# Jaureguy760/HaploHyped-VarAwareML

Measured on AMD Instinct MI355X. Metric: variants/sec encode+compress, 3M-variant x 2.5k-sample VCF, higher is better.
Workload: dtype u8

## Files before the change

### haplohyped_varawareml_amd/csrc/api.hip

```cpp
#include "common.h"
#include <chrono>
#include <vector>
#include <stdarg.h>
#include <stdio.h>
#include <string.h>
#include <stdlib.h>

static thread_local char g_err[512] = "";

void hhgt_set_error(const char *fmt, ...)
{
    va_list ap;
    va_start(ap, fmt);
    vsnprintf(g_err, sizeof(g_err), fmt, ap);
    va_end(ap);
}

extern "C" const char *hhgt_last_error(void) { return g_err; }
extern "C" const char *hhgt_version(void) { return "hhgt 0.1 (gfx950)"; }

extern "C" int hhgt_device_count(void)
{
    int n = 0;
    if (hipGetDeviceCount(&n) != hipSuccess) return 0;
    return n;
}

int DevBuf::ensure(size_t bytes)
{
    if (bytes <= cap) return HHGT_OK;
    if (p) {
        hipFree(p);
        p = nullptr;
        cap = 0;
    }
    size_t want = bytes + bytes / 8 + 256;
    static const bool dbg = getenv("HHGT_ALLOC_DEBUG") != nullptr;
    const auto t0 = std::chrono::steady_clock::now();
    hipError_t e = hipMalloc(&p, want);
    if (dbg)
        fprintf(stderr, "[alloc] %.3f ms  hipMalloc %zu took %.3f ms\n", std::chrono::duration<double>(t0.time_since_epoch()).count() * 1e3,
                want, std::chrono::duration<double>(std::chrono::steady_clock::now() - t0).count() * 1e3);
    if (e != hipSuccess) {
        p = nullptr;
        hhgt_set_error("hipMalloc(%zu) failed: %s", want, hipGetErrorString(e));
        return HHGT_ERR_HIP;
    }
    cap = want;
    return HHGT_OK;
}

void DevBuf::release()
{
    if (p) hipFree(p);
    p = nullptr;
    cap = 0;
}

#define TRY(expr)                      \
    do {                               \
        int _rc = (expr);              \
        if (_rc != HHGT_OK) return _rc; \
    } while (0)

int EncodeWs::ensure_index(uint32_t n_regions)
{
    TRY(slots.ensure((size_t)n_regions * INDEX_CAP * 4));
    TRY(counts.ensure((size_t)n_regions * 4));
    TRY(prefix.ensure(((size_t)n_regions + 1) * 4));
    return ensure_scan(n_regions);
}

int EncodeWs::ensure_lines(uint32_t max_lines)
{
    const size_t nl4 = ((size_t)max_lines + 1) * 4;
    TRY(nl.ensure(nl4));
    TRY(ensure_scan(max_lines));
    for (DevBuf &b : line) TRY(b.ensure(nl4));
    return ensure_runs();
}

int EncodeWs::ensure_scan(uint64_t n) { return scan_tmp.ensure(2 * scan_tmp_elems(n) * 4); }

int EncodeWs::ensure_runs()
{
    TRY(run_first.ensure(MAX_CHROM_RUNS * 8));
    TRY(run_names.ensure(MAX_CHROM_RUNS * 32));
    return result.ensure(sizeof(hhgt_encode_result));
}

int hhgt_ctx::CodecWs::ensure(uint64_t n_chunks, uint32_t nblocks, uint32_t nwaves, size_t slot)
{
    const uint64_t n_streams = n_chunks * nblocks * nwaves;
    TRY(lz_scratch.ensure((size_t)n_streams * slot));
    TRY(lz_csize.ensure((size_t)n_streams * 4));
    TRY(fr_bsize.ensure((size_t)n_chunks * nblocks * 4));
    TRY(fr_csize.ensure(((size_t)n_chunks + 1) * 8));
    return fr_flags.ensure((size_t)n_chunks * 4);
}

template <typename Launch>
static int timed(hhgt_ctx *c, hipStream_t st, int stage, Launch launch)
{
    StageTimer t(c, st, stage);
    TRY(launch());
    t.stop();
    return HHGT_OK;
}

extern "C" int hhgt_ctx_create(int device, hhgt_ctx **out)
{
    if (!out) return HHGT_ERR_ARG;
    *out = nullptr;
    int n = hhgt_device_count();
    if (n <= 0 || device < 0 || device >= n) {
        hhgt_set_error("no usable HIP device (count=%d, requested=%d): libhhgt has no CPU path", n, device);
        return HHGT_ERR_NO_DEVICE;
    }
    HIP_TRY(hipSetDevice(device));
    hhgt_ctx *c = new hhgt_ctx();
    c->device = device;
    int rc = HHGT_OK;
    hipError_t e = hipGetDeviceProperties(&c->prop, device);
    if (e != hipSuccess) {
        hhgt_set_error("hipGetDeviceProperties failed: %s", hipGetErrorString(e));
        rc = HHGT_ERR_HIP;
    } else if (strncmp(c->prop.gcnArchName, "gfx950", 6) != 0) {
        hhgt_set_error("device %d is %s; libhhgt carries gfx950 code objects only", device, c->prop.gcnArchName);
        rc = HHGT_ERR_NO_DEVICE;
    }
    if (rc == HHGT_OK && (e = hipHostMalloc(reinterpret_cast<void **>(&c->h_counters), sizeof(DevCounters), hipHostMallocDefault)) != hipSuccess) {
        hhgt_set_error("hipHostMalloc failed: %s", hipGetErrorString(e));
        rc = HHGT_ERR_HIP;
    }
    if (rc == HHGT_OK && (e = hipHostMalloc(reinterpret_cast<void **>(&c->h_result_pinned), sizeof(hhgt_encode_result), hipHostMallocDefault)) != hipSuccess) {
        hhgt_set_error("hipHostMalloc failed: %s", hipGetErrorString(e));
        rc = HHGT_ERR_HIP;
    }
    if (rc == HHGT_OK) rc = c->counters.ensure(sizeof(DevCounters));
    if (rc != HHGT_OK) {
        hhgt_ctx_destroy(c);
        return rc;
    }
    *out = c;
    return HHGT_OK;
}

extern "C" void hhgt_ctx_destroy(hhgt_ctx *c)
{
    if (!c) return;
    hipSetDevice(c->device);
    hipDeviceSynchronize();
    c->enc.each([](DevBuf &b) { b.release(); });
    DevBuf *bufs[] = {&c->counters, &c->cursor, &c->dec_bad, &c->oh_ovl, &c->oh_lut, &c->crc_x2n, &c->ld_bits};
    for (DevBuf *b : bufs) b->release();
    for (auto &w : c->cw) {
        DevBuf *wb[] = {&w.lz_scratch, &w.lz_csize, &w.lz_flags, &w.fr_bsize, &w.fr_csize, &w.fr_flags};
        for (DevBuf *b : wb) b->release();
        if (w.lz_done) hipEventDestroy(w.lz_done);
        if (w.fr_done) hipEventDestroy(w.fr_done);
    }
    if (c->h_counters) hipHostFree(c->h_counters);
    if (c->h_result_pinned) hipHostFree(c->h_result_pinned);
    for (auto &p : c->pending) {
        hipEventDestroy(p.a);
        hipEventDestroy(p.b);
    }
    for (auto e : c->event_pool) hipEventDestroy(e);
    delete c;
}

static hipEvent_t get_event(hhgt_ctx *c)
{
    if (!c->event_pool.empty()) {
        hipEvent_t e = c->event_pool.back();
        c->event_pool.pop_back();
        return e;
    }
    hipEvent_t e;
    hipEventCreate(&e);
    return e;
}

StageTimer::StageTimer(hhgt_ctx *c, hipStream_t s, int stage_) : ctx(c), st(s), stage(stage_)
{
    if (ctx->profiling) {
        a = get_event(ctx);
        b = get_event(ctx);
        hipEventRecord(a, st);
    }
}

void StageTimer::stop()
{
    if (a) {
        hipEventRecord(b, st);
        ctx->pending.push_back({stage, a, b});
        a = b = nullptr;
    }
}

int hhgt_profile_collect(hhgt_ctx *c)
{
    for (auto &p : c->pending) {
        hipEventSynchronize(p.b);
        float ms = 0.f;
        if (hipEventElapsedTime(&ms, p.a, p.b) == hipSuccess) {
            c->stage_ms[p.stage] += ms;
            c->stage_launches[p.stage] += 1;
        }
        c->event_pool.push_back(p.a);
        c->event_pool.push_back(p.b);
    }
    c->pending.clear();
    return HHGT_OK;
}

extern "C" int hhgt_profile_enable(hhgt_ctx *c, int on)
{
    if (!c) return HHGT_ERR_ARG;
    c->profiling = on ? 1 : 0;
    return HHGT_OK;
}

extern "C" int hhgt_profile_reset(hhgt_ctx *c)
{
    if (!c) return HHGT_ERR_ARG;
    hhgt_profile_collect(c);
    for (int i = 0; i < HHGT_N_STAGES; ++i) {
        c->stage_ms[i] = 0;
        c->stage_launches[i] = 0;
    }
    return HHGT_OK;
}

extern "C" int hhgt_profile_read(hhgt_ctx *c, double *ms, uint64_t *launches)
{
    if (!c) return HHGT_ERR_ARG;
    hhgt_profile_collect(c);
    for (int i = 0; i < HHGT_N_STAGES; ++i) {
        if (ms) ms[i] = c->stage_ms[i];
        if (launches) launches[i] = c->stage_launches[i];
    }
    return HHGT_OK;
}

static int make_layout(const hhgt_layout *lay, LayoutDev *L)
{
    if (!lay || lay->n_samples < 0) {
        hhgt_set_error("layout: bad n_samples");
        return HHGT_ERR_ARG;
    }
    L->S = (uint32_t)lay->n_samples;
    L->v_capacity = lay->v_capacity;
    L->ring = 0;
    L->pad_ = 0;
    if (lay->ring < 0 || (lay->ring > 0 && (lay->vc <= 0 || lay->v_capacity != (uint64_t)lay->ring * (uint64_t)lay->vc))) {
        hhgt_set_error("layout: a ring needs vc > 0 and v_capacity == ring * vc");
        return HHGT_ERR_ARG;
    }
    L->ring = (uint32_t)lay->ring;
    if (lay->vc == 0) {
        L->Vc = lay->v_capacity ? lay->v_capacity : TILE_V;
    } else {
        L->Vc = (uint64_t)lay->vc;
    }
    if (L->Vc % TILE_V) {
        hhgt_set_error("layout: variants per chunk (%llu) must be a multiple of %d (dense: v_capacity)",
                       (unsigned long long)L->Vc, TILE_V);
        return HHGT_ERR_ARG;
    }
    if (lay->v_capacity % L->Vc) {
        hhgt_set_error("layout: v_capacity must be a multiple of vc");
        return HHGT_ERR_ARG;
    }
    if (lay->sc == 0) {
        L->Sc = L->S ? L->S : 1;
        L->sc_log2 = 31;
        L->n_sc = 1;
    } else {
        uint32_t sc = (uint32_t)lay->sc;
        if (sc & (sc - 1)) {
            hhgt_set_error("layout: sc must be a power of two");
            return HHGT_ERR_ARG;
        }
        L->Sc = sc;
        uint32_t lg = 0;
        while ((1u << lg) < sc) ++lg;
        L->sc_log2 = lg;
        L->n_sc = (L->S + sc - 1) / sc;
        if (L->n_sc == 0) L->n_sc = 1;
    }
    return HHGT_OK;
}

extern "C" uint64_t hhgt_layout_bytes(const hhgt_layout *lay)
{
    LayoutDev L;
    if (make_layout(lay, &L) != HHGT_OK) return 0;
    return (uint64_t)L.n_sc * L.Sc * L.v_capacity * 2ull;
}

extern "C" uint64_t hhgt_layout_offset(const hhgt_layout *lay, uint32_t s, uint64_t v)
{
    LayoutDev L;
    if (make_layout(lay, &L) != HHGT_OK) return ~0ull;
    return layout_offset(L, s, v);
}

static int parse_region_host(const char *region, RegionFilter *rf)
{
    memset(rf, 0, sizeof(*rf));
    if (!region || !*region) return HHGT_OK;
    const char *colon = strrchr(region, ':');
    size_t clen = strlen(region);
    if (colon && colon[1] >= '0' && colon[1] <= '9') {
        char *p;
        long long b = strtoll(colon + 1, &p, 10), e = 0x7fffffffffffffffLL;
        while (*p == ',') p++;
        if (*p == '-' && p[1]) e = strtoll(p + 1, &p, 10);
        clen = (size_t)(colon - region);
        rf->has_range = 1;
        rf->beg = b;
        rf->end = e;
    }
    if (clen == 0 || clen >= sizeof(rf->contig)) {
        hhgt_set_error("region '%s': contig name empty or longer than 63 bytes", region);
        return HHGT_ERR_ARG;
    }
    memcpy(rf->contig, region, clen);
    rf->contig_len = (int)clen;
    return HHGT_OK;
}

__global__ void k_encode_finish(DevCounters *cnt, uint64_t *cursor, const uint64_t *__restrict__ run_first,
                                const uint8_t *__restrict__ run_names, uint64_t v_capacity, hhgt_encode_result *res)
{
    const uint32_t t = threadIdx.x;
    const uint64_t before = *cursor;
    const uint64_t kept = cnt->n_kept;
    __syncthreads();
    if (t == 0) {
        *cursor = before + kept;
        cnt->cursor_after = before + kept;
        res->stats.n_lines = cnt->n_lines;
        res->stats.n_records = cnt->n_records;
        res->stats.n_kept = kept;
        res->stats.n_drop_region = cnt->n_drop_region;
        res->stats.n_drop_filter = cnt->n_drop_filter;
        res->stats.n_haploid_padded = cnt->n_haploid;
        res->stats.n_malformed = cnt->n_malformed;
        res->stats.n_general_lines = cnt->n_general;
        res->stats.n_chrom_runs = cnt->n_chrom_runs;
        res->cursor_before = before;
        res->cursor_after = before + kept;
        res->n_lines_over = cnt->err_lines;
        res->err_density = cnt->err_density;
        res->v_capacity = v_capacity;
        res->done = 1u;
        res->reserved = cnt->n_other > 0xFFFFFFFFull ? 0xFFFFFFFFu : (uint32_t)cnt->n_other;
    }
    const uint64_t n_runs = cnt->n_chrom_runs;
    if (t < HHGT_RESULT_RUNS) res->run_first[t] = t < n_runs ? run_first[t] : 0ull;
    for (uint32_t q = t; q < HHGT_RESULT_RUNS * 32u; q += blockDim.x)
        res->run_names[q >> 5][q & 31u] = (q >> 5) < n_runs ? (char)run_names[q] : 0;
    __syncthreads();
    if (t < sizeof(DevCounters) / 8u) reinterpret_cast<unsigned long long *>(cnt)[t] = 0ull;
}

__global__ void k_set_u64(uint64_t *p, uint64_t v) { *p = v; }

static int encode_check_args(hhgt_ctx *c, const void *d_text, uint64_t nbytes, const hhgt_layout *lay, LayoutDev *L,
                             const char *region, RegionFilter *rf, void *d_G)
{
    TRY(make_layout(lay, L));
    if (nbytes >= 0xFFFFFFF0ull) {
        hhgt_set_error("encode: text block of %llu bytes; split it below 4 GiB at a line boundary",
                       (unsigned long long)nbytes);
        return HHGT_ERR_ARG;
    }
    if (nbytes && (!d_text || (reinterpret_cast<uintptr_t>(d_text) & 15u))) {
        hhgt_set_error("encode: d_text must be a 16-byte aligned device pointer");
        return HHGT_ERR_ARG;
    }
    if (L->S > 0 && !d_G) {
        hhgt_set_error("encode: d_G is NULL");
        return HHGT_ERR_ARG;
    }
    const int rc = parse_region_host(region, rf);
    rf->keep_multi = c->keep_multi;
    return rc;
}

static uint32_t index_regions(uint64_t nbytes) { return (uint32_t)((nbytes + 1 + INDEX_REGION - 1) / INDEX_REGION); }

static int encode_stage_index(hhgt_ctx *c, const uint8_t *text, uint64_t nbytes, uint32_t n_regions, uint32_t min_line, uint32_t S,
                              DevCounters *cnt, hipStream_t st)
{
    EncodeWs &w = c->enc;
    TRY(w.ensure_index(n_regions));
    TRY(launch_index_newlines(text, nbytes, w.slots.as<uint32_t>(), w.counts.as<uint32_t>(), n_regions, min_line, S, c->index_mode, cnt, st));
    TRY(launch_scan_exclusive_u32_pair(w.counts.as<uint32_t>(), w.prefix.as<uint32_t>(), nullptr, nullptr, n_regions,
                                       w.scan_tmp.as<uint32_t>(), w.scan_tmp.cap / 4, st));
    return HHGT_OK;
}

static int encode_stage_rest(hhgt_ctx *c, const uint8_t *text, uint64_t nbytes, uint32_t n_regions, uint32_t max_lines,
                             const RegionFilter &rf, const LayoutDev &L, const uint64_t *d_cursor, void *d_G, void *d_P, uint32_t *d_start, uint32_t *d_stop,
                             uint8_t *d_ref, uint8_t *d_alt, DevCounters *cnt, hipStream_t st)
{
    EncodeWs &w = c->enc;
    TRY(w.ensure_lines(max_lines));
    const uint32_t *nl = w.nl.as<uint32_t>(), *d_nlines = w.prefix.as<uint32_t>() + n_regions;
    uint32_t *scan_tmp = w.scan_tmp.as<uint32_t>();
    const LineCols l = w.line_cols();
    const KeptCols k = w.kept_cols();
    TRY(timed(c, st, HHGT_STAGE_INDEX, [&] {
        return launch_compact_newlines(w.slots.as<uint32_t>(), w.counts.as<uint32_t>(), w.prefix.as<uint32_t>(), n_regions,
                                       w.nl.as<uint32_t>(), max_lines, st);
    }));
    if (max_lines == 0) return HHGT_OK;
    TRY(timed(c, st, HHGT_STAGE_FIXED, [&] {
        TRY(launch_parse_fixed(text, nbytes, nl, d_nlines, max_lines, rf, L.S, l, c->index_mode, cnt, st));
        TRY(launch_scan_exclusive_u32_pair(l.keep, l.kidx, l.cnew, l.crun, max_lines, scan_tmp, w.scan_tmp.cap / 4, st));
        return launch_compact_kept(text, nbytes, nl, d_nlines, max_lines, l, k, MAX_CHROM_RUNS, d_cursor, L.v_capacity, L.ring,
                                   d_start, d_stop, d_ref, d_alt, cnt, d_P != nullptr, st);
    }));
    if (L.S == 0) return HHGT_OK;
    TRY(timed(c, st, HHGT_STAGE_ENCODE, [&] {
        return d_P ? launch_encode_planes(text, nbytes, k.soff, k.meta, max_lines, d_cursor, L, static_cast<uint8_t *>(d_P),
                                          static_cast<int8_t *>(d_G), k.redo_list, k.redo_flag, cnt, st)
                   : launch_encode_tiles(text, nbytes, k.soff, k.meta, max_lines, d_cursor, L, static_cast<int8_t *>(d_G),
                                         k.redo_list, k.redo_flag, cnt, st);
    }));
    return timed(c, st, HHGT_STAGE_GENERAL, [&] {
        return launch_encode_general(text, nbytes, k.soff, k.lend, k.meta, k.redo_list, d_cursor, L, static_cast<int8_t *>(d_G),
                                     static_cast<uint8_t *>(d_P), cnt, c->prop.multiProcessorCount, st);
    });
}

static int encode_finish(hhgt_ctx *c, uint64_t *d_cursor, const LayoutDev &L, DevCounters *cnt, hipStream_t st)
{
    TRY(c->enc.ensure_runs());
    const KeptCols k = c->enc.kept_cols();
    hipLaunchKernelGGL(k_encode_finish, dim3(1), dim3(256), 0, st, cnt, d_cursor, k.run_first, k.run_names,
                       L.ring ? 0ull : L.v_capacity, c->enc.result.as<hhgt_encode_result>());
    HIP_TRY(hipGetLastError());
    return HHGT_OK;
}

extern "C" int hhgt_encode_result_status(const hhgt_encode_result *r)
{
    if (!r) return HHGT_ERR_ARG;
    if (!r->done) {
        hhgt_set_error("encode: the result record is not complete yet (synchronise the stream first)");
        return HHGT_ERR_ARG;
    }
    if (r->err_density) {
        hhgt_set_error("encode: more than %u newlines inside one %u-byte region (not VCF text)", INDEX_CAP, INDEX_REGION);
        return HHGT_ERR_LINE_DENSITY;
    }
    if (r->n_lines_over) {
        hhgt_set_error("encode: %llu lines beyond max_lines were not encoded", (unsigned long long)r->n_lines_over);
        return HHGT_ERR_CAPACITY;
    }
    if (r->stats.n_malformed) {
        hhgt_set_error("Error parsing VCF file: %llu malformed record(s) (too few columns, bad POS, FORMAT without GT)",
                       (unsigned long long)r->stats.n_malformed);
        return HHGT_ERR_MALFORMED;
    }
    if (r->v_capacity && r->cursor_after > r->v_capacity) {
        hhgt_set_error("encode: %llu kept records at v_base %llu exceed v_capacity %llu",
                       (unsigned long long)r->stats.n_kept, (unsigned long long)r->cursor_before,
                       (unsigned long long)r->v_capacity);
        return HHGT_ERR_CAPACITY;
    }
    if (r->stats.n_chrom_runs > MAX_CHROM_RUNS) {
        hhgt_set_error("encode: %llu CHROM runs in one text block, more than the limit of %u (a run starts at every change of CHROM "
                       "and behind every empty or header line)",
                       (unsigned long long)r->stats.n_chrom_runs, MAX_CHROM_RUNS);
        return HHGT_ERR_CAPACITY;
    }
    return HHGT_OK;
}

static void empty_result(hhgt_encode_result *r)
{
    memset(r, 0, sizeof(*r));
    r->done = 1u;
}

static int planes_check_layout(const LayoutDev &L)
{
    if (L.Vc % 4096ull) {
        hhgt_set_error("planes: variants per chunk (%llu; dense: v_capacity) must be a multiple of 4096", (unsigned long long)L.Vc);
        return HHGT_ERR_ARG;
    }
    return HHGT_OK;
}

extern "C" uint64_t hhgt_planes_bytes(const hhgt_layout *lay)
{
    LayoutDev L;
    if (make_layout(lay, &L) != HHGT_OK || planes_check_layout(L) != HHGT_OK) return 0;
    return (uint64_t)L.n_sc * L.Sc * L.v_capacity / 2ull;
}

static int planes_columns(const hhgt_layout *lay, uint32_t col0, uint32_t n_cols, LayoutDev *L, PlanesGeom *pg)
{
    TRY(make_layout(lay, L));
    TRY(planes_check_layout(*L));
    if ((uint64_t)col0 + n_cols > L->v_capacity / L->Vc) {
        hhgt_set_error("planes: columns [%u, %u) outside the layout's %llu", col0, col0 + n_cols, (unsigned long long)(L->v_capacity / L->Vc));
        return HHGT_ERR_ARG;
    }
    *pg = planes_geom(*L, col0);
    return HHGT_OK;
}

static int pad_tail_begin(hhgt_ctx *c, const void *d_buf, const hhgt_layout *lay, bool planes, LayoutDev *L)
{
    if (!c || !d_buf) return HHGT_ERR_ARG;
    HIP_TRY(hipSetDevice(c->device));
    TRY(make_layout(lay, L));
    return planes ? planes_check_layout(*L) : HHGT_OK;
}

static int pad_tail_range(const LayoutDev &L, uint64_t v_end, uint64_t vcol_end)
{
    if (v_end > L.v_capacity || vcol_end > L.v_capacity / L.Vc) {
        hhgt_set_error("pad_tail: range outside the layout");
        return HHGT_ERR_ARG;
    }
    return HHGT_OK;
}

static int encode_async_impl(hhgt_ctx *c, const void *d_text, uint64_t nbytes, const char *region, const hhgt_layout *lay,
                             uint64_t *d_cursor, uint32_t max_lines, void *d_G, void *d_P, bool planes, uint32_t *d_start,
                             uint32_t *d_stop, uint8_t *d_ref, uint8_t *d_alt, hhgt_encode_result *h_result, void *stream)
{
    if (!c || !d_cursor) return HHGT_ERR_ARG;
    hipStream_t st = reinterpret_cast<hipStream_t>(stream);
    HIP_TRY(hipSetDevice(c->device));
    LayoutDev L;
    RegionFilter rf;
    TRY(encode_check_args(c, d_text, nbytes, lay, &L, region, &rf, planes ? d_P : d_G));
    if (planes) TRY(planes_check_layout(L));
    const uint8_t *text = static_cast<const uint8_t *>(d_text);
    DevCounters *cnt = c->counters.as<DevCounters>();
    if (!c->counters_clean) HIP_TRY(hipMemsetAsync(cnt, 0, sizeof(DevCounters), st));
    c->counters_clean = false;
    const uint32_t n_regions = index_regions(nbytes);
    if (nbytes) {
        TRY(timed(c, st, HHGT_STAGE_INDEX, [&] { return encode_stage_index(c, text, nbytes, n_regions, L.S ? 2u * L.S + 17u : 0u, L.S, cnt, st); }));
        TRY(encode_stage_rest(c, text, nbytes, n_regions, max_lines, rf, L, d_cursor, d_G, planes ? d_P : nullptr, d_start, d_stop, d_ref,
                              d_alt, cnt, st));
    }
    TRY(encode_finish(c, d_cursor, L, cnt, st));
    c->counters_clean = true;
    if (h_result) {
        h_result->done = 0u;
        HIP_TRY(hipMemcpyAsync(h_result, c->enc.result.p, sizeof(hhgt_encode_result), hipMemcpyDeviceToHost, st));
    }
    return HHGT_OK;
}

extern "C" int hhgt_encode_text_async(hhgt_ctx *c, const void *d_text, uint64_t nbytes, const char *region,
                                      const hhgt_layout *lay, uint64_t *d_cursor, uint32_t max_lines, void *d_G,
                                      uint32_t *d_start, uint32_t *d_stop, uint8_t *d_ref, uint8_t *d_alt,
                                      hhgt_encode_result *h_result, void *stream)
{
    return encode_async_impl(c, d_text, nbytes, region, lay, d_cursor, max_lines, d_G, nullptr, false, d_start, d_stop, d_ref, d_alt,
                             h_result, stream);
}

extern "C" int hhgt_encode_text_planes_async(hhgt_ctx *c, const void *d_text, uint64_t nbytes, const char *region,
                                             const hhgt_layout *lay, uint64_t *d_cursor, uint32_t max_lines, void *d_P, void *d_G,
                                             uint32_t *d_start, uint32_t *d_stop, uint8_t *d_ref, uint8_t *d_alt,
                                             hhgt_encode_result *h_result, void *stream)
{
    return encode_async_impl(c, d_text, nbytes, region, lay, d_cursor, max_lines, d_G, d_P, true, d_start, d_stop, d_ref, d_alt,
                             h_result, stream);
}

extern "C" int hhgt_pad_tail_planes(hhgt_ctx *c, const hhgt_layout *lay, uint64_t v_end, uint64_t vcol_begin, uint64_t vcol_end,
                                    void *d_P, void *stream)
{
    LayoutDev L;
    TRY(pad_tail_begin(c, d_P, lay, true, &L));
    TRY(pad_tail_range(L, v_end, vcol_end));
    return launch_pad_tail_planes(L, v_end, vcol_begin, vcol_end, static_cast<uint8_t *>(d_P), reinterpret_cast<hipStream_t>(stream));
}

extern "C" int hhgt_pad_tail_planes_cursor(hhgt_ctx *c, const hhgt_layout *lay, const uint64_t *d_cursor, void *d_P, void *stream)
{
    LayoutDev L;
    if (!d_cursor) return HHGT_ERR_ARG;
    TRY(pad_tail_begin(c, d_P, lay, true, &L));
    return launch_pad_tail_planes_cursor(L, d_cursor, static_cast<uint8_t *>(d_P), reinterpret_cast<hipStream_t>(stream));
}

extern "C" int hhgt_planes_expand(hhgt_ctx *c, const hhgt_layout *lay, const void *d_P, const void *d_G, uint32_t col0, uint32_t n_cols,
                                  void *d_out, void *stream)
{
    if (!c || !d_P || !d_out) return HHGT_ERR_ARG;
    HIP_TRY(hipSetDevice(c->device));
    LayoutDev L;
    PlanesGeom pg;
    TRY(planes_columns(lay, col0, n_cols, &L, &pg));
    if (n_cols == 0) return HHGT_OK;
    return launch_planes_expand(L, static_cast<const uint8_t *>(d_P), static_cast<const uint8_t *>(d_G), col0, n_cols,
                                static_cast<uint8_t *>(d_out), reinterpret_cast<hipStream_t>(stream));
}

static int encode_text_once(hhgt_ctx *c, const void *d_text, uint64_t nbytes, const char *region, const hhgt_layout *lay, uint64_t v_base,
                            void *d_G, uint32_t *d_start, uint32_t *d_stop, uint8_t *d_ref, uint8_t *d_alt, hhgt_encode_stats *stats,
                            void *stream);

extern "C" int hhgt_encode_text(hhgt_ctx *c, const void *d_text, uint64_t nbytes, const char *region,
                                const hhgt_layout *lay, uint64_t v_base, void *d_G, uint32_t *d_start,
                                uint32_t *d_stop, uint8_t *d_ref, uint8_t *d_alt, hhgt_encode_stats *stats,
                                void *stream)
{
    int rc = encode_text_once(c, d_text, nbytes, region, lay, v_base, d_G, d_start, d_stop, d_ref, d_alt, stats, stream);
    if (rc == HHGT_ERR_MALFORMED && c && lay && lay->n_samples >= 760) {
        const int mode = c->index_mode < 0 ? index_mode_default() : c->index_mode;
        if (mode > 0) {
            const int saved = c->index_mode;
            c->index_mode = 0;
            rc = encode_text_once(c, d_text, nbytes, region, lay, v_base, d_G, d_start, d_stop, d_ref, d_alt, stats, stream);
            c->index_mode = saved;
        }
    }
    return rc;
}

static int encode_text_once(hhgt_ctx *c, const void *d_text, uint64_t nbytes, const char *region, const hhgt_layout *lay, uint64_t v_base,
                            void *d_G, uint32_t *d_start, uint32_t *d_stop, uint8_t *d_ref, uint8_t *d_alt, hhgt_encode_stats *stats,
                            void *stream)
{
    if (!c) return HHGT_ERR_ARG;
    hipStream_t st = reinterpret_cast<hipStream_t>(stream);
    HIP_TRY(hipSetDevice(c->device));
    if (stats) memset(stats, 0, sizeof(*stats));
    LayoutDev L;
    RegionFilter rf;
    TRY(encode_check_args(c, d_text, nbytes, lay, &L, region, &rf, d_G));
    c->run_first_kept.clear();
    c->run_names_host.clear();
    if (nbytes == 0) return HHGT_OK;

    const uint8_t *text = static_cast<const uint8_t *>(d_text);
    DevCounters *cnt = c->counters.as<DevCounters>();
    TRY(c->cursor.ensure(8));
    HIP_TRY(hipMemsetAsync(cnt, 0, sizeof(DevCounters), st));
    c->counters_clean = false;
    hipLaunchKernelGGL(k_set_u64, dim3(1), dim3(1), 0, st, c->cursor.as<uint64_t>(), v_base);
    const uint32_t n_regions = index_regions(nbytes);
    uint32_t n_lines = 0;
    {
        StageTimer t(c, st, HHGT_STAGE_INDEX);
        TRY(encode_stage_index(c, text, nbytes, n_regions, L.S ? 2u * L.S + 17u : 0u, L.S, cnt, st));
        c->h_counters->n_lines = 0;
        c->h_counters->err_density = 0;
        HIP_TRY(hipMemcpyAsync(&c->h_counters->n_lines, c->enc.prefix.as<uint32_t>() + n_regions, 4,
                               hipMemcpyDeviceToHost, st));
        HIP_TRY(hipMemcpyAsync(&c->h_counters->err_density, &cnt->err_density, 8, hipMemcpyDeviceToHost, st));
        HIP_TRY(hipStreamSynchronize(st));
        t.stop();
        n_lines = (uint32_t)(c->h_counters->n_lines & 0xFFFFFFFFull);
        if (c->h_counters->err_density) {
            hhgt_set_error("encode: more than %u newlines inside one %u-byte region (not VCF text)", INDEX_CAP,
                           INDEX_REGION);
            return HHGT_ERR_LINE_DENSITY;
        }
    }
    if (stats) stats->n_lines = n_lines;
    if (n_lines == 0) return HHGT_OK;
    TRY(encode_stage_rest(c, text, nbytes, n_regions, n_lines, rf, L, c->cursor.as<uint64_t>(), d_G, nullptr, d_start, d_stop, d_ref,
                          d_alt, cnt, st));
    TRY(encode_finish(c, c->cursor.as<uint64_t>(), L, cnt, st));
    c->counters_clean = true;
    hhgt_encode_result *hr = &c->h_result;
    hr->done = 0u;
    HIP_TRY(hipMemcpyAsync(c->h_result_pinned, c->enc.result.p, sizeof(hhgt_encode_result), hipMemcpyDeviceToHost, st));
    HIP_TRY(hipStreamSynchronize(st));
    *hr = *c->h_result_pinned;
    if (stats) *stats = hr->stats;
    TRY(hhgt_encode_result_status(hr));
    const uint32_t n_runs = (uint32_t)hr->stats.n_chrom_runs;
    if (n_runs) {
        std::vector<uint64_t> first(n_runs);
        std::vector<char> names((size_t)n_runs * 32);
        if (n_runs <= HHGT_RESULT_RUNS) {
            memcpy(first.data(), hr->run_first, n_runs * 8);
            memcpy(names.data(), hr->run_names, (size_t)n_runs * 32);
        } else {
            HIP_TRY(hipMemcpy(first.data(), c->enc.run_first.p, (size_t)n_runs * 8, hipMemcpyDeviceToHost));
            HIP_TRY(hipMemcpy(names.data(), c->enc.run_names.p, (size_t)n_runs * 32, hipMemcpyDeviceToHost));
        }
        for (uint32_t r = 0; r < n_runs; ++r) {
            c->run_first_kept.push_back(first[r]);
            c->run_names_host.emplace_back(names.data() + (size_t)r * 32, strnlen(names.data() + (size_t)r * 32, 31));
        }
    }
    return HHGT_OK;
}

extern "C" int hhgt_encode_chrom_runs(hhgt_ctx *c, uint32_t max_runs, uint64_t *first_kept, char *names,
                                      uint32_t *n_runs)
{
    if (!c || !n_runs) return HHGT_ERR_ARG;
    uint32_t n = (uint32_t)c->run_first_kept.size();
    *n_runs = n;
    if (n > max_runs) n = max_runs;
    for (uint32_t r = 0; r < n; ++r) {
        if (first_kept) first_kept[r] = c->run_first_kept[r];
        if (names) {
            memset(names + (size_t)r * 32, 0, 32);
            size_t l = c->run_names_host[r].size() < 31 ? c->run_names_host[r].size() : 31;
            memcpy(names + (size_t)r * 32, c->run_names_host[r].data(), l);
        }
    }
    return HHGT_OK;
}

extern "C" int hhgt_pad_tail(hhgt_ctx *c, const hhgt_layout *lay, uint64_t v_end, uint64_t vcol_begin,
                             uint64_t vcol_end, void *d_G, void *stream)
{
    LayoutDev L;
    TRY(pad_tail_begin(c, d_G, lay, false, &L));
    TRY(pad_tail_range(L, v_end, vcol_end));
    return launch_pad_tail(L, v_end, vcol_begin, vcol_end, static_cast<int8_t *>(d_G),
                           reinterpret_cast<hipStream_t>(stream));
}

extern "C" int hhgt_pad_tail_cursor(hhgt_ctx *c, const hhgt_layout *lay, const uint64_t *d_cursor, void *d_G, void *stream)
{
    LayoutDev L;
    if (!d_cursor) return HHGT_ERR_ARG;
    TRY(pad_tail_begin(c, d_G, lay, false, &L));
    return launch_pad_tail_cursor(L, d_cursor, static_cast<int8_t *>(d_G), reinterpret_cast<hipStream_t>(stream));
}

static int check_codec_args(uint64_t chunk_nbytes, int typesize, int blocksize, int format)
{
    if (typesize < 1 || typesize > 255 || blocksize < 16 || blocksize > 65536 || blocksize % typesize ||
        chunk_nbytes == 0 || chunk_nbytes >= 0x7fffffffull || (format != HHGT_BLOSC1 && format != HHGT_BLOSC2)) {
        hhgt_set_error("compress: bad arguments (chunk_nbytes=%llu typesize=%d blocksize=%d format=%d)",
                       (unsigned long long)chunk_nbytes, typesize, blocksize, format);
        return HHGT_ERR_ARG;
    }
    return HHGT_OK;
}

static int effective_blocksize(uint64_t chunk_nbytes, int typesize, int blocksize)
{
    if ((uint64_t)blocksize > chunk_nbytes) {
        blocksize = (int)chunk_nbytes;
        if (typesize > 1 && blocksize >= typesize) blocksize -= blocksize % typesize;
    }
    return blocksize > 0 ? blocksize : 1;
}

static int check_decode_block(int typesize, int blocksize)
{
    if (blocksize > 65536) {
        hhgt_set_error("decode: block of %d bytes x typesize %d does not fit LDS (blocks of at most 65536 bytes)",
                       blocksize, typesize);
        return HHGT_ERR_ARG;
    }
    return HHGT_OK;
}

static void codec_geometry(uint64_t chunk_nbytes, int typesize, int blocksize, uint32_t *nblocks, uint32_t *nwaves,
                           size_t *slot_bytes)
{
    const bool split = typesize >= 2 && typesize <= 16 && blocksize / typesize >= 128;
    *nblocks = (uint32_t)((chunk_nbytes + blocksize - 1) / blocksize);
    *nwaves = split ? (uint32_t)typesize : 1u;
    size_t max_stream = split ? (size_t)blocksize / typesize : (size_t)blocksize;
    if (split && chunk_nbytes % blocksize && chunk_nbytes % blocksize > max_stream) max_stream = chunk_nbytes % blocksize;
    *slot_bytes = lz4_slot_bytes((int)max_stream);
}

extern "C" uint64_t hhgt_compress_bound(uint64_t n_chunks, uint64_t chunk_nbytes, int typesize, int blocksize)
{
    if (check_codec_args(chunk_nbytes, typesize, blocksize, HHGT_BLOSC2) != HHGT_OK) return 0;
    return n_chunks * (chunk_nbytes + 32);
}

static int compress_impl(hhgt_ctx *c, const void *d_src, const void *d_planes, PlanesGeom pg, uint64_t n_chunks, uint64_t chunk_nbytes,
                         int typesize, int blocksize, int format, void *d_dst, uint64_t dst_cap,
                         uint64_t *d_chunk_off, uint64_t *total_bytes, void *stream)
{
    if (!c || (!d_src && !d_planes) || !d_dst || !d_chunk_off) return HHGT_ERR_ARG;
    hipStream_t st = reinterpret_cast<hipStream_t>(stream);
    HIP_TRY(hipSetDevice(c->device));
    TRY(check_codec_args(chunk_nbytes, typesize, blocksize, format));
    if (total_bytes) *total_bytes = 0;
    if (n_chunks == 0) return HHGT_OK;
    if (!total_bytes && dst_cap < n_chunks * (chunk_nbytes + 32)) {
        hhgt_set_error("compress: the asynchronous form (total_bytes == NULL) needs dst_cap >= hhgt_compress_bound() = %llu, got %llu",
                       (unsigned long long)(n_chunks * (chunk_nbytes + 32)), (unsigned long long)dst_cap);
        return HHGT_ERR_CAPACITY;
    }
    blocksize = effective_blocksize(chunk_nbytes, typesize, blocksize);
    uint32_t nblocks, nwaves;
    size_t slot;
    codec_geometry(chunk_nbytes, typesize, blocksize, &nblocks, &nwaves, &slot);
    hipStream_t fst = c->frame_stream ? c->frame_stream : st;
    hhgt_ctx::CodecWs &w = c->cw[c->frame_stream ? (c->cmp_seq++ & 1u) : 0u];
    TRY(w.ensure(n_chunks, nblocks, nwaves, slot));
    if (w.fr_pending) {
        HIP_TRY(hipStreamWaitEvent(st, w.fr_done, 0));
        w.fr_pending = false;
    }
    TRY(timed(c, st, HHGT_STAGE_LZ4, [&] {
        if (!w.lz_flags.p) {
            TRY(w.lz_flags.ensure(4));
            HIP_TRY(hipMemsetAsync(w.lz_flags.p, 0, 4, st));
        }
        if (++w.lz_tag == 0) w.lz_tag = 1;
        return launch_lz4_blocks(static_cast<const uint8_t *>(d_src), static_cast<const uint8_t *>(d_planes), pg, n_chunks, chunk_nbytes,
                                 typesize, blocksize, w.lz_scratch.as<uint8_t>(), slot, w.lz_csize.as<uint32_t>(), c->clevel,
                                 w.lz_flags.as<uint32_t>(), w.lz_tag, st);
    }));
    if (fst != st) {
        if (!w.lz_done) HIP_TRY(hipEventCreateWithFlags(&w.lz_done, hipEventDisableTiming));
        if (!w.fr_done) HIP_TRY(hipEventCreateWithFlags(&w.fr_done, hipEventDisableTiming));
        HIP_TRY(hipEventRecord(w.lz_done, st));
        HIP_TRY(hipStreamWaitEvent(fst, w.lz_done, 0));
    }
    TRY(timed(c, fst, HHGT_STAGE_FRAME, [&] {
        return launch_frame(w.lz_scratch.as<uint8_t>(), slot, w.lz_csize.as<uint32_t>(), static_cast<const uint8_t *>(d_src),
                            static_cast<const uint8_t *>(d_planes), pg, n_chunks, chunk_nbytes, typesize, blocksize, format,
                            w.fr_bsize.as<uint32_t>(), w.fr_csize.as<uint64_t>(), static_cast<uint8_t *>(d_dst), dst_cap, d_chunk_off,
                            w.fr_flags.as<uint32_t>(), fst);
    }));
    if (fst != st) {
        HIP_TRY(hipEventRecord(w.fr_done, fst));
        w.fr_pending = true;
        if (total_bytes) HIP_TRY(hipStreamWaitEvent(st, w.fr_done, 0));
    }
    if (total_bytes) {
        uint64_t tot = 0;
        HIP_TRY(hipMemcpyAsync(&tot, d_chunk_off + n_chunks, 8, hipMemcpyDeviceToHost, st));
        HIP_TRY(hipStreamSynchronize(st));
        *total_bytes = tot;
        if (tot > dst_cap) {
            hhgt_set_error("compress: need %llu bytes, dst_cap is %llu", (unsigned long long)tot,
                           (unsigned long long)dst_cap);
            return HHGT_ERR_CAPACITY;
        }
    }
    return HHGT_OK;
}

extern "C" int hhgt_compress_chunks(hhgt_ctx *c, const void *d_src, uint64_t n_chunks, uint64_t chunk_nbytes,
                                    int typesize, int blocksize, int format, void *d_dst, uint64_t dst_cap,
                                    uint64_t *d_chunk_off, uint64_t *total_bytes, void *stream)
{
    if (!d_src) return HHGT_ERR_ARG;
    return compress_impl(c, d_src, nullptr, PlanesGeom{0, 0, 0, 0}, n_chunks, chunk_nbytes, typesize, blocksize, format, d_dst, dst_cap,
                         d_chunk_off, total_bytes, stream);
}

extern "C" int hhgt_compress_planes(hhgt_ctx *c, const hhgt_layout *lay, const void *d_P, const void *d_G, uint32_t col0, uint32_t n_cols,
                                    int format, void *d_dst, uint64_t dst_cap, uint64_t *d_chunk_off, uint64_t *total_bytes,
                                    void *stream)
{
    if (!c || !d_P) return HHGT_ERR_ARG;
    LayoutDev L;
    PlanesGeom pg;
    TRY(planes_columns(lay, col0, n_cols, &L, &pg));
    const uint64_t chunk_nbytes = (uint64_t)L.Sc * L.Vc * 2ull, col_bytes = chunk_nbytes * L.n_sc;
    const uint8_t *g = d_G ? static_cast<const uint8_t *>(d_G) + (uint64_t)col0 * col_bytes : nullptr;
    return compress_impl(c, g, d_P, pg, (uint64_t)n_cols * L.n_sc, chunk_nbytes, 2, 8192, format, d_dst, dst_cap, d_chunk_off, total_bytes,
                         stream);
}

extern "C" int hhgt_reserve(hhgt_ctx *c, uint64_t text_bytes, uint32_t max_lines, uint64_t n_chunks, uint64_t chunk_nbytes, int typesize,
                            int blocksize)
{
    if (!c) return HHGT_ERR_ARG;
    HIP_TRY(hipSetDevice(c->device));
    if (text_bytes) {
        const uint32_t n_regions = index_regions(text_bytes);
        TRY(c->enc.ensure_scan(n_regions > max_lines ? n_regions : max_lines));
        TRY(c->enc.ensure_index(n_regions));
        TRY(c->enc.ensure_lines(max_lines));
    }
    if (n_chunks) {
        TRY(check_codec_args(chunk_nbytes, typesize, blocksize, HHGT_BLOSC2));
        blocksize = effective_blocksize(chunk_nbytes, typesize, blocksize);
        uint32_t nblocks, nwaves;
        size_t slot;
        codec_geometry(chunk_nbytes, typesize, blocksize, &nblocks, &nwaves, &slot);
        TRY(c->cw[0].ensure(n_chunks, nblocks, nwaves, slot));
    }
    return HHGT_OK;
}

extern "C" int hhgt_set_clevel(hhgt_ctx *c, int clevel)
{
    if (!c || clevel < 1 || clevel > 9) {
        hhgt_set_error("clevel must be 1..9");
        return HHGT_ERR_ARG;
    }
    c->clevel = clevel;
    return HHGT_OK;
}

extern "C" int hhgt_stream_create(hhgt_ctx *c, int kind, void **out)
{
    if (!c || !out || (kind != HHGT_STREAM_ENCODE && kind != HHGT_STREAM_COMPRESS && kind != HHGT_STREAM_FRAME)) {
        hhgt_set_error("hhgt_stream_create: bad arguments");
        return HHGT_ERR_ARG;
    }
    HIP_TRY(hipSetDevice(c->device));
    hipStream_t st = nullptr;
    if (kind == HHGT_STREAM_FRAME) {
        HIP_TRY(hipStreamCreateWithFlags(&st, hipStreamNonBlocking));
    } else if (kind == HHGT_STREAM_ENCODE) {
        int lo = 0, hi = 0;
        HIP_TRY(hipDeviceGetStreamPriorityRange(&lo, &hi));
        HIP_TRY(hipStreamCreateWithPriority(&st, hipStreamNonBlocking, hi));
    } else {
        const uint32_t n_cu = (uint32_t)c->prop.multiProcessorCount;
        uint32_t use = n_cu >= 128u ? (n_cu * 3u / 4u) / 32u * 32u : n_cu;
        if (const char *e = getenv("HHGT_COMPRESS_CUS")) {
            const int v = atoi(e);
            use = v <= 0 || (uint32_t)v >= n_cu ? n_cu : (uint32_t)v;
        }
        if (use >= n_cu) {
            HIP_TRY(hipStreamCreateWithFlags(&st, hipStreamNonBlocking));
        } else {
            std::vector<uint32_t> mask((n_cu + 31u) / 32u, 0u);
            for (uint32_t i = n_cu - use; i < n_cu; ++i) mask[i >> 5] |= 1u << (i & 31u);
            if (hipExtStreamCreateWithCUMask(&st, (uint32_t)mask.size(), mask.data()) != hipSuccess) {
                (void)hipGetLastError();
                st = nullptr;
                HIP_TRY(hipStreamCreateWithFlags(&st, hipStreamNonBlocking));
            }
        }
    }
    *out = st;
    return HHGT_OK;
}

extern "C" int hhgt_set_frame_stream(hhgt_ctx *c, void *stream)
{
    if (!c) return HHGT_ERR_ARG;
    HIP_TRY(hipSetDevice(c->device));
    if (c->frame_stream) HIP_TRY(hipStreamSynchronize(c->frame_stream));
    for (auto &w : c->cw) w.fr_pending = false;
    c->frame_stream = reinterpret_cast<hipStream_t>(stream);
    return HHGT_OK;
}

extern "C" int hhgt_stream_destroy(hhgt_ctx *c, void *stream)
{
    if (!c) return HHGT_ERR_ARG;
    if (stream) {
        HIP_TRY(hipSetDevice(c->device));
        if (reinterpret_cast<hipStream_t>(stream) == c->frame_stream) TRY(hhgt_set_frame_stream(c, nullptr));
        HIP_TRY(hipStreamDestroy(reinterpret_cast<hipStream_t>(stream)));
    }
    return HHGT_OK;
}

extern "C" int hhgt_set_index_mode(hhgt_ctx *c, int mode)
{
    if (!c || mode < -1 || mode > 2) {
        hhgt_set_error("index mode must be -1 (default), 0 (scan), 1 (hop) or 2 (walk)");
        return HHGT_ERR_ARG;
    }
    c->index_mode = mode;
    return HHGT_OK;
}

extern "C" int hhgt_set_keep_multiallelic(hhgt_ctx *c, int on)
{
    if (!c) return HHGT_ERR_ARG;
    c->keep_multi = on ? 1 : 0;
    return HHGT_OK;
}

__global__ void k_count_nonzero_u32(const uint32_t *__restrict__ v, uint64_t n, unsigned long long *out)
{
    uint64_t i = (uint64_t)blockIdx.x * blockDim.x + threadIdx.x;
    const unsigned long long m = __ballot(i < n && v[i] != 0u);
    if ((threadIdx.x & 63u) == 0u && m) atomicAdd(out, (unsigned long long)__builtin_popcountll(m));
}

extern "C" int hhgt_inflate_members(hhgt_ctx *c, const void *d_src, uint64_t src_bytes, const uint64_t *d_comp_off,
                                    const uint32_t *d_comp_len, const uint64_t *d_out_off, const uint32_t *d_isize,
                                    uint64_t n_members, void *d_dst, uint64_t dst_bytes, const uint32_t *d_crc32,
                                    uint32_t *d_status, uint64_t *n_bad, void *stream)
{
    if (!c || !d_src || !d_comp_off || !d_comp_len || !d_out_off || !d_isize || !d_status || (!d_dst && dst_bytes))
        return HHGT_ERR_ARG;
    hipStream_t st = reinterpret_cast<hipStream_t>(stream);
    HIP_TRY(hipSetDevice(c->device));
    if (n_bad) *n_bad = 0;
    if (n_members == 0) return HHGT_OK;
    if (d_crc32 && !c->crc_x2n_ready) {
        uint32_t t[32];
        crc32_x2n_table(t);
        TRY(c->crc_x2n.ensure(sizeof(t)));
        HIP_TRY(hipMemcpy(c->crc_x2n.p, t, sizeof(t), hipMemcpyHostToDevice));
        c->crc_x2n_ready = true;
    }
    TRY(timed(c, st, HHGT_STAGE_INFLATE, [&] {
        return launch_inflate(static_cast<const uint8_t *>(d_src), src_bytes, d_comp_off, d_comp_len, d_out_off, d_isize, n_members,
                              static_cast<uint8_t *>(d_dst), dst_bytes, d_status, d_crc32, c->crc_x2n.as<uint32_t>(), st);
    }));
    if (n_bad) {
        TRY(c->dec_bad.ensure(8));
        HIP_TRY(hipMemsetAsync(c->dec_bad.p, 0, 8, st));
        hipLaunchKernelGGL(k_count_nonzero_u32, dim3((uint32_t)((n_members + 255) / 256)), dim3(256), 0, st, d_status,
                           n_members, c->dec_bad.as<unsigned long long>());
        HIP_TRY(hipGetLastError());
        uint64_t nb = 0;
        HIP_TRY(hipMemcpyAsync(&nb, c->dec_bad.p, 8, hipMemcpyDeviceToHost, st));
        HIP_TRY(hipStreamSynchronize(st));
        *n_bad = nb;
    }
    return HHGT_OK;
}

template <typename Launch>
static int with_bad_counter(hhgt_ctx *c, hipStream_t st, uint64_t *n_bad, Launch launch)
{
    TRY(c->dec_bad.ensure(8));
    HIP_TRY(hipMemsetAsync(c->dec_bad.p, 0, 8, st));
    TRY(timed(c, st, HHGT_STAGE_DECODE, [&] { return launch(c->dec_bad.as<unsigned long long>()); }));
    if (n_bad) {
        uint64_t nb = 0;
        HIP_TRY(hipMemcpyAsync(&nb, c->dec_bad.p, 8, hipMemcpyDeviceToHost, st));
        HIP_TRY(hipStreamSynchronize(st));
        *n_bad = nb;
    }
    return HHGT_OK;
}

extern "C" int hhgt_decompress_chunks(hhgt_ctx *c, const void *d_src, const uint64_t *d_chunk_off, uint64_t n_chunks,
                                      uint64_t chunk_nbytes, int typesize, int blocksize, void *d_dst,
                                      uint64_t *n_bad, void *stream)
{
    if (!c || !d_src || !d_dst || !d_chunk_off) return HHGT_ERR_ARG;
    hipStream_t st = reinterpret_cast<hipStream_t>(stream);
    HIP_TRY(hipSetDevice(c->device));
    TRY(check_decode_block(typesize, blocksize));
    TRY(check_codec_args(chunk_nbytes, typesize, blocksize, HHGT_BLOSC2));
    if (n_bad) *n_bad = 0;
    if (n_chunks == 0) return HHGT_OK;
    blocksize = effective_blocksize(chunk_nbytes, typesize, blocksize);
    return with_bad_counter(c, st, n_bad, [&](unsigned long long *d_bad) {
        return launch_decode(static_cast<const uint8_t *>(d_src), d_chunk_off, n_chunks, chunk_nbytes, typesize, blocksize,
                             static_cast<uint8_t *>(d_dst), d_bad, st);
    });
}

extern "C" int hhgt_decompress_blocks(hhgt_ctx *c, const hhgt_block_sel *d_sel, uint32_t n_sel, uint64_t chunk_nbytes,
                                      int typesize, int blocksize, void *d_dst, uint64_t *n_bad, void *stream)
{
    if (!c || (n_sel && (!d_sel || !d_dst))) {
        hhgt_set_error("decompress_blocks: null %s", !c ? "context" : !d_sel ? "selection array" : "destination");
        return HHGT_ERR_ARG;
    }
    hipStream_t st = reinterpret_cast<hipStream_t>(stream);
    HIP_TRY(hipSetDevice(c->device));
    TRY(check_decode_block(typesize, blocksize));
    TRY(check_codec_args(chunk_nbytes, typesize, blocksize, HHGT_BLOSC2));
    if (n_bad) *n_bad = 0;
    if (n_sel == 0) return HHGT_OK;
    blocksize = effective_blocksize(chunk_nbytes, typesize, blocksize);
    return with_bad_counter(c, st, n_bad, [&](unsigned long long *d_bad) {
        return launch_decode_sel(d_sel, n_sel, chunk_nbytes, typesize, blocksize, static_cast<uint8_t *>(d_dst), d_bad, st);
    });
}

static int check_row_kernel_args(const char *who, uint32_t sc, uint32_t vc, int typesize, int blocksize)
{
    if (typesize != 2) {
        hhgt_set_error("%s: typesize %d (only 2: one diploid int8 call)", who, typesize);
        return HHGT_ERR_ARG;
    }
    if (sc < 1 || sc > 64 || vc < 1) {
        hhgt_set_error("%s: chunk of %u samples x %u variants (1 to 64 samples)", who, sc, vc);
        return HHGT_ERR_ARG;
    }
    TRY(check_codec_args((uint64_t)sc * vc * 2u, typesize, blocksize, HHGT_BLOSC2));
    if (blocksize > 8192 || ((uint64_t)vc * 2u) % (uint64_t)blocksize) {
        hhgt_set_error("%s: blocksize %d does not cut a row of %u variants into whole blocks of at most 8192 bytes", who,
                       blocksize, vc);
        return HHGT_ERR_ARG;
    }
    return HHGT_OK;
}

template <typename Launch>
static int run_row_kernel(const char *who, const char *out, hhgt_ctx *c, const void *d_sel, uint32_t n_sel, const void *d_out,
                          uint32_t sc, uint32_t vc, int typesize, int blocksize, uint64_t *n_bad, void *stream, Launch launch)
{
    if (!c || (n_sel && (!d_sel || !d_out))) {
        hhgt_set_error("%s: null %s", who, !c ? "context" : !d_sel ? "selection array" : out);
        return HHGT_ERR_ARG;
    }
    TRY(check_row_kernel_args(who, sc, vc, typesize, blocksize));
    hipStream_t st = reinterpret_cast<hipStream_t>(stream);
    HIP_TRY(hipSetDevice(c->device));
    if (n_bad) *n_bad = 0;
    if (n_sel == 0) return HHGT_OK;
    return with_bad_counter(c, st, n_bad, [&](unsigned long long *d_bad) { return launch(d_bad, st); });
}

extern "C" int hhgt_count_alleles(hhgt_ctx *c, const hhgt_count_sel *d_sel, uint32_t n_sel, uint32_t sc, uint32_t vc,
                                  int typesize, int blocksize, uint32_t *d_counts, uint64_t n_out, uint64_t *n_bad,
                                  void *stream)
{
    return run_row_kernel("count_alleles", "counts", c, d_sel, n_sel, d_counts, sc, vc, typesize, blocksize, n_bad, stream,
                          [&](unsigned long long *d_bad, hipStream_t st) {
                              return launch_count_alleles(d_sel, n_sel, sc, vc, blocksize, d_counts, n_out, d_bad, st);
                          });
}

extern "C" int hhgt_count_samples(hhgt_ctx *c, const hhgt_sample_sel *d_sel, uint32_t n_sel, uint32_t sc, uint32_t vc,
                                  int typesize, int blocksize, const uint32_t *d_vmask, uint64_t vmask_words,
                                  uint32_t *d_counts, uint64_t n_out, uint64_t *n_bad, void *stream)
{
    return run_row_kernel("count_samples", "counts", c, d_sel, n_sel, d_counts, sc, vc, typesize, blocksize, n_bad, stream,
                          [&](unsigned long long *d_bad, hipStream_t st) {
                              return launch_count_samples(d_sel, n_sel, sc, vc, blocksize, d_vmask, vmask_words, d_counts,
                                                          n_out, d_bad, st);
                          });
}

extern "C" int hhgt_genotype_planes(hhgt_ctx *c, const hhgt_plane_sel *d_sel, uint32_t n_sel, uint32_t sc, uint32_t vc,
                                    int typesize, int blocksize, const uint32_t *d_vmask, uint64_t vmask_words,
                                    uint32_t *d_planes, uint64_t n_rows, uint64_t row_words, uint64_t *n_bad,
                                    void *stream)
{
    return run_row_kernel("genotype_planes", "planes", c, d_sel, n_sel, d_planes, sc, vc, typesize, blocksize, n_bad, stream,
                          [&](unsigned long long *d_bad, hipStream_t st) {
                              return launch_genotype_planes(d_sel, n_sel, sc, vc, blocksize, d_vmask, vmask_words, d_planes,
                                                            n_rows, row_words, d_bad, st);
                          });
}

template <typename Launch>
static int run_plane_kernel(const char *who, int stage, hhgt_ctx *c, const char *null_arg, const char *misaligned, uint64_t n_rows,
                            uint64_t row_words, uint64_t w_lo, uint64_t w_hi, uint64_t row_limit, void *stream, Launch launch)
{
    const bool work = n_rows && w_lo < w_hi;
    if (!c || (work && null_arg)) {
        hhgt_set_error("%s: null %s", who, !c ? "context" : null_arg);
        return HHGT_ERR_ARG;
    }
    if (w_lo > w_hi || w_hi > row_words || n_rows > row_limit) {
        hhgt_set_error("%s: words [%llu, %llu) of rows of %llu words, %llu rows", who, (unsigned long long)w_lo,
                       (unsigned long long)w_hi, (unsigned long long)row_words, (unsigned long long)n_rows);
        return HHGT_ERR_ARG;
    }
    if (misaligned) {
        hhgt_set_error("%s: %s", who, misaligned);
        return HHGT_ERR_ARG;
    }
    hipStream_t st = reinterpret_cast<hipStream_t>(stream);
    HIP_TRY(hipSetDevice(c->device));
    if (!work) return HHGT_OK;
    return timed(c, st, stage, [&] { return launch(st); });
}

static bool off_alignment(const void *p, uintptr_t align) { return reinterpret_cast<uintptr_t>(p) & (align - 1u); }

extern "C" int hhgt_pair_counts(hhgt_ctx *c, const uint32_t *d_planes, uint64_t n_rows, uint64_t row_words, uint64_t w_lo,
                                uint64_t w_hi, uint32_t *d_table, void *stream)
{
    return run_plane_kernel("pair_counts", HHGT_STAGE_PAIRS, c, !d_planes ? "planes" : !d_table ? "table" : nullptr,
                            off_alignment(d_table, 16) ? "the table must be 16-byte aligned" : nullptr, n_rows, row_words, w_lo, w_hi,
                            64ull * 65535ull, stream, [&](hipStream_t st) {
                                return launch_pair_counts(d_planes, (uint32_t)n_rows, row_words, w_lo, w_hi, d_table, st);
                            });
}

extern "C" int hhgt_grm(hhgt_ctx *c, const uint32_t *d_planes, uint64_t n_rows, uint64_t row_words, uint64_t w_lo, uint64_t w_hi,
                        const float *d_z, double *d_table, void *stream)
{
    return run_plane_kernel("grm", HHGT_STAGE_GRM, c, !d_planes ? "planes" : !d_z ? "weights" : !d_table ? "table" : nullptr,
                            off_alignment(d_table, 8) || off_alignment(d_z, 16)
                                ? "the table must be 8-byte aligned, the weights 16-byte aligned" : nullptr,
                            n_rows, row_words, w_lo, w_hi, 64ull * 65535ull, stream, [&](hipStream_t st) {
                                return launch_grm(d_planes, (uint32_t)n_rows, row_words, w_lo, w_hi, d_z, d_table, st);
                            });
}

extern "C" int hhgt_variant_planes(hhgt_ctx *c, const uint32_t *d_planes, uint64_t n_rows, uint64_t row_words, uint64_t w_lo,
                                   uint64_t w_hi, uint32_t *d_vplanes, void *stream)
{
    return run_plane_kernel("variant_planes", HHGT_STAGE_LD_TRANSPOSE, c, !d_planes ? "planes" : !d_vplanes ? "variant planes" : nullptr,
                            nullptr, n_rows, row_words, w_lo, w_hi, 256ull * 65535ull, stream, [&](hipStream_t st) {
                                return launch_variant_planes(d_planes, (uint32_t)n_rows, row_words, w_lo, w_hi, d_vplanes, st);
                            });
}

static int check_ld_args(const char *who, hhgt_ctx *c, uint32_t window, const double *r2, const char *null_arg, const uint32_t *d_table)
{
    if (window < 1u || window > 1024u || (r2 && !(*r2 >= 0.0 && *r2 <= 1.0))) {
        if (r2)
            hhgt_set_error("%s: window %u, r2 %g (1 to 1024, 0 to 1)", who, window, *r2);
        else
            hhgt_set_error("%s: window %u (1 to 1024)", who, window);
        return HHGT_ERR_ARG;
    }
    if (!c || null_arg) {
        hhgt_set_error("%s: null %s", who, !c ? "context" : null_arg);
        return HHGT_ERR_ARG;
    }
    if (off_alignment(d_table, 32)) {
        hhgt_set_error("%s: the table must be 32-byte aligned", who);
        return HHGT_ERR_ARG;
    }
    return HHGT_OK;
}

extern "C" int hhgt_ld_counts(hhgt_ctx *c, const uint32_t *d_vplanes, uint64_t n_var, uint64_t sw, uint32_t window,
                              uint32_t *d_table, void *stream)
{
    const bool work = n_var && sw;
    TRY(check_ld_args("ld_counts", c, window, nullptr, !work ? nullptr : !d_vplanes ? "variant planes" : !d_table ? "table" : nullptr, d_table));
    hipStream_t st = reinterpret_cast<hipStream_t>(stream);
    HIP_TRY(hipSetDevice(c->device));
    if (!work) return HHGT_OK;
    return timed(c, st, HHGT_STAGE_LD, [&] { return launch_ld_counts(d_vplanes, n_var, sw, window, d_table, st); });
}

extern "C" int hhgt_ld_prune(hhgt_ctx *c, const uint32_t *d_table, uint64_t n_var, uint32_t window, double r2,
                             uint8_t *d_keep, void *stream)
{
    TRY(check_ld_args("ld_prune", c, window, &r2, !n_var ? nullptr : !d_table ? "table" : !d_keep ? "keep flags" : nullptr, d_table));
    hipStream_t st = reinterpret_cast<hipStream_t>(stream);
    HIP_TRY(hipSetDevice(c->device));
    if (!n_var) return HHGT_OK;
    TRY(c->ld_bits.ensure((size_t)n_var * ld_walk_words(window) * sizeof(uint64_t)));
    uint64_t *bits = c->ld_bits.as<uint64_t>();
    TRY(timed(c, st, HHGT_STAGE_LD_PRUNE, [&] { return launch_ld_exceeds(d_table, n_var, window, r2, bits, st); }));
    return timed(c, st, HHGT_STAGE_LD_WALK, [&] { return launch_ld_walk(bits, n_var, window, d_keep, st); });
}

extern "C" int hhgt_assoc_sums(hhgt_ctx *c, const uint32_t *d_vplanes, uint64_t n_var, uint64_t sw, const double *d_w,
                               uint32_t n_cols, double *d_sums, void *stream)
{
    if (n_cols < 1u || n_cols > 64u) {
        hhgt_set_error("assoc_sums: %u columns (1 to 64)", n_cols);
        return HHGT_ERR_ARG;
    }
    const bool reads = n_var && sw;
    const char *null_arg = !n_var ? nullptr : !d_sums ? "sums" : !reads ? nullptr : !d_vplanes ? "variant planes" : !d_w ? "weights" : nullptr;
    if (!c || null_arg) {
        hhgt_set_error("assoc_sums: null %s", !c ? "context" : null_arg);
        return HHGT_ERR_ARG;
    }
    if (off_alignment(d_w, 8) || off_alignment(d_sums, 8)) {
        hhgt_set_error("assoc_sums: the weights and the sums must be 8-byte aligned");
        return HHGT_ERR_ARG;
    }
    hipStream_t st = reinterpret_cast<hipStream_t>(stream);
    HIP_TRY(hipSetDevice(c->device));
    if (!n_var) return HHGT_OK;
    return timed(c, st, HHGT_STAGE_ASSOC, [&] { return launch_assoc_sums(d_vplanes, n_var, sw, d_w, n_cols, d_sums, st); });
}
```

### haplohyped_varawareml_amd/csrc/common.h

```cpp
#pragma once
#include <hip/hip_runtime.h>
#include <stdint.h>
#include <stddef.h>
#include <string>
#include <vector>
#include "../../include/hhgt.h"

#define HHGT_WAVE 64
#ifdef HHGT_ENC_PRIO
#define HHGT_WAVE_PRIO() __builtin_amdgcn_s_setprio(HHGT_ENC_PRIO)
#else
#define HHGT_WAVE_PRIO()
#endif

#ifdef __HIPCC__
__device__ __forceinline__ uint32_t wave_scan_sum_dpp(uint32_t x, uint32_t lane)
{
    x += (uint32_t)__builtin_amdgcn_update_dpp(0, (int)x, 0x111, 0xf, 0xf, false);
    x += (uint32_t)__builtin_amdgcn_update_dpp(0, (int)x, 0x112, 0xf, 0xf, false);
    x += (uint32_t)__builtin_amdgcn_update_dpp(0, (int)x, 0x114, 0xf, 0xf, false);
    x += (uint32_t)__builtin_amdgcn_update_dpp(0, (int)x, 0x118, 0xf, 0xf, false);
    const uint32_t t0 = (uint32_t)__builtin_amdgcn_readlane((int)x, 15);
    const uint32_t t1 = (uint32_t)__builtin_amdgcn_readlane((int)x, 31) + t0;
    const uint32_t t2 = (uint32_t)__builtin_amdgcn_readlane((int)x, 47) + t1;
    const uint32_t row = lane >> 4;
    return x + (row == 0u ? 0u : (row == 1u ? t0 : (row == 2u ? t1 : t2)));
}
#endif

void hhgt_set_error(const char *fmt, ...);
#define HIP_TRY(expr)                                                                      \
    do {                                                                                   \
        hipError_t _e = (expr);                                                            \
        if (_e != hipSuccess) {                                                            \
            hhgt_set_error("%s failed: %s (%s:%d)", #expr, hipGetErrorString(_e), __FILE__, \
                           __LINE__);                                                      \
            return HHGT_ERR_HIP;                                                           \
        }                                                                                  \
    } while (0)

enum : uint32_t {
    LF_RECORD = 1u,
    LF_KEEP = 2u,
    LF_FAST = 4u,
    LF_MALFORMED = 8u,
    LF_DROP_REGION = 16u,
    LF_DROP_FILTER = 32u,
    LF_CHROM_NEW = 64u,
};

struct DevCounters {
    unsigned long long n_lines;
    unsigned long long n_records;
    unsigned long long n_kept;
    unsigned long long n_drop_region;
    unsigned long long n_drop_filter;
    unsigned long long n_haploid;
    unsigned long long n_malformed;
    unsigned long long n_general;
    unsigned long long n_chrom_runs;
    unsigned long long err_density;
    unsigned long long err_lines;
    unsigned long long cursor_after;
    unsigned long long n_other;
    unsigned long long pad[3];
};

#define MAX_CHROM_RUNS 4096u

struct RegionFilter {
    char contig[64];
    int contig_len;
    int has_range;
    long long beg, end;
    int keep_multi;
};

#define INDEX_REGION 16384u
#define INDEX_CAP 1024u

#define TILE_V 128
#define TILE_S 256

struct LayoutDev {
    uint32_t S;
    uint32_t sc_log2;
    uint32_t n_sc;
    uint32_t Sc;
    uint64_t Vc;
    uint64_t v_capacity;
    uint32_t ring;
    uint32_t pad_;
};

#define PL_TILE 256u
struct PlanesGeom {
    uint32_t S_pad;
    uint32_t bpr;
    uint32_t tpc;
    uint32_t col0;
};
static inline __host__ __device__ uint64_t planes_piece(const PlanesGeom &g, uint64_t col, uint32_t tile, uint32_t kp, uint32_t row)
{
    return ((((col * g.tpc + tile) * 4ull + kp) * g.S_pad) + row) * 32ull;
}
static inline __host__ __device__ PlanesGeom planes_geom(const LayoutDev &L, uint32_t col0)
{
    PlanesGeom g;
    g.S_pad = L.n_sc * L.Sc;
    g.bpr = (uint32_t)(L.Vc >> 12);
    g.tpc = (uint32_t)(L.Vc / PL_TILE);
    g.col0 = col0;
    return g;
}
static inline __host__ __device__ void planes_block(const PlanesGeom &g, uint64_t id, uint64_t *col, uint32_t *row, uint32_t *bi)
{
    const uint64_t per_col = (uint64_t)g.S_pad * g.bpr;
    const uint64_t c = id / per_col;
    const uint32_t rem = (uint32_t)(id - c * per_col);
    *col = g.col0 + c;
    *row = rem / g.bpr;
    *bi = rem - (rem / g.bpr) * g.bpr;
}

struct DevBuf {
    void *p = nullptr;
    size_t cap = 0;
    int ensure(size_t bytes);
    void release();
    template <typename T> T *as() const { return reinterpret_cast<T *>(p); }
};

struct LineCols {
    uint32_t *soff, *lend, *pos, *refalt, *flags, *keep, *kidx, *cnew, *crun;
};
struct KeptCols {
    uint32_t *soff, *lend, *meta, *redo_list, *redo_flag;
    uint64_t *run_first;
    uint8_t *run_names;
};

struct EncodeWs {
    DevBuf slots, counts, prefix, nl, scan_tmp;
    enum { L_SOFF, L_LEND, L_POS, L_REFALT, L_FLAGS, L_KEEP, L_KIDX, L_CNEW, L_CRUN, K_SOFF, K_LEND, K_META, REDO_LIST, REDO_FLAG, N_LINE };
    DevBuf line[N_LINE];
    DevBuf run_first, run_names;
    DevBuf result;
    int ensure_index(uint32_t n_regions);
    int ensure_lines(uint32_t max_lines);
    int ensure_scan(uint64_t n);
    int ensure_runs();
    template <typename F> void each(F f)
    {
        for (DevBuf *b : {&slots, &counts, &prefix, &nl, &scan_tmp, &run_first, &run_names, &result}) f(*b);
        for (DevBuf &b : line) f(b);
    }
    uint32_t *col(int i) const { return line[i].as<uint32_t>(); }
    LineCols line_cols() const
    {
        LineCols l;
        l.soff = col(L_SOFF), l.lend = col(L_LEND), l.pos = col(L_POS), l.refalt = col(L_REFALT), l.flags = col(L_FLAGS);
        l.keep = col(L_KEEP), l.kidx = col(L_KIDX), l.cnew = col(L_CNEW), l.crun = col(L_CRUN);
        return l;
    }
    KeptCols kept_cols() const
    {
        KeptCols k;
        k.soff = col(K_SOFF), k.lend = col(K_LEND), k.meta = col(K_META), k.redo_list = col(REDO_LIST), k.redo_flag = col(REDO_FLAG);
        k.run_first = run_first.as<uint64_t>(), k.run_names = run_names.as<uint8_t>();
        return k;
    }
};

struct hhgt_ctx {
    int device = 0;
    hipDeviceProp_t prop;
    EncodeWs enc;
    DevBuf counters;
    DevBuf cursor;
    struct CodecWs {
        DevBuf lz_scratch, lz_csize, lz_flags, fr_bsize, fr_csize, fr_flags;
        uint32_t lz_tag = 0;
        hipEvent_t lz_done = nullptr, fr_done = nullptr;
        bool fr_pending = false;
        int ensure(uint64_t n_chunks, uint32_t nblocks, uint32_t nwaves, size_t slot);
    } cw[2];
    uint64_t cmp_seq = 0;
    hipStream_t frame_stream = nullptr;
    DevBuf dec_bad, oh_ovl, oh_lut, crc_x2n;
    DevBuf ld_bits;
    bool crc_x2n_ready = false;
    DevCounters *h_counters = nullptr;
    hhgt_encode_result *h_result_pinned = nullptr;
    hhgt_encode_result h_result;
    std::vector<uint64_t> run_first_kept;
    std::vector<std::string> run_names_host;
    int clevel = 5;
    int keep_multi = 0;
    int index_mode = -1;
    bool counters_clean = false;
    int profiling = 0;
    double stage_ms[HHGT_N_STAGES] = {0};
    uint64_t stage_launches[HHGT_N_STAGES] = {0};
    struct Pending { int stage; hipEvent_t a, b; };
    std::vector<Pending> pending;
    std::vector<hipEvent_t> event_pool;
};

struct StageTimer {
    hhgt_ctx *ctx;
    hipStream_t st;
    int stage;
    hipEvent_t a = nullptr, b = nullptr;
    StageTimer(hhgt_ctx *c, hipStream_t s, int stage_);
    void stop();
};
int hhgt_profile_collect(hhgt_ctx *ctx);

int launch_scan_exclusive_u32(const uint32_t *d_in, uint32_t *d_out, uint64_t n, uint32_t *d_tmp,
                              size_t tmp_elems, hipStream_t st);
int launch_scan_exclusive_u32_pair(const uint32_t *in_a, uint32_t *out_a, const uint32_t *in_b, uint32_t *out_b, uint64_t n,
                                   uint32_t *d_tmp, size_t tmp_elems, hipStream_t st);
size_t scan_tmp_elems(uint64_t n);

int launch_index_newlines(const uint8_t *d_text, uint64_t n, uint32_t *d_slots, uint32_t *d_counts,
                          uint32_t n_regions, uint32_t min_line, uint32_t S, int mode, DevCounters *d_cnt, hipStream_t st);
int index_mode_default();
int launch_compact_newlines(const uint32_t *d_slots, const uint32_t *d_counts, const uint32_t *d_prefix,
                            uint32_t n_regions, uint32_t *d_nl, uint32_t max_lines, hipStream_t st);
int launch_parse_fixed(const uint8_t *d_text, uint64_t n, const uint32_t *d_nl, const uint32_t *d_nlines,
                       uint32_t max_lines, const RegionFilter &region, uint32_t S, const LineCols &l, int mode,
                       DevCounters *d_cnt, hipStream_t st);
int launch_compact_kept(const uint8_t *d_text, uint64_t n, const uint32_t *d_nl, const uint32_t *d_nlines, uint32_t max_lines,
                        const LineCols &l, const KeptCols &k, uint32_t max_runs, const uint64_t *d_cursor, uint64_t v_capacity,
                        uint32_t ring, uint32_t *d_start, uint32_t *d_stop, uint8_t *d_ref, uint8_t *d_alt, DevCounters *d_cnt,
                        bool strided, hipStream_t st);

int launch_encode_tiles(const uint8_t *d_text, uint64_t n, const uint32_t *k_soff, const uint32_t *k_meta,
                        uint32_t n_lines_bound, const uint64_t *d_cursor, LayoutDev lay, int8_t *d_G,
                        uint32_t *redo_list, uint32_t *redo_flag, DevCounters *d_cnt, hipStream_t st);
int launch_encode_general(const uint8_t *d_text, uint64_t n, const uint32_t *k_soff, const uint32_t *k_lend,
                          const uint32_t *k_meta, const uint32_t *redo_list, const uint64_t *d_cursor, LayoutDev lay,
                          int8_t *d_G, uint8_t *d_P, DevCounters *d_cnt, int n_cu, hipStream_t st);
int launch_encode_planes(const uint8_t *d_text, uint64_t n, const uint32_t *k_soff, const uint32_t *k_meta,
                         uint32_t n_lines_bound, const uint64_t *d_cursor, LayoutDev lay, uint8_t *d_P, int8_t *d_G,
                         uint32_t *redo_list, uint32_t *redo_flag, DevCounters *d_cnt, hipStream_t st);
int launch_pad_tail_planes(LayoutDev lay, uint64_t v_end, uint64_t vcol_begin, uint64_t vcol_end, uint8_t *d_P, hipStream_t st);
int launch_pad_tail_planes_cursor(LayoutDev lay, const uint64_t *d_cursor, uint8_t *d_P, hipStream_t st);
int launch_planes_expand(LayoutDev lay, const uint8_t *d_P, const uint8_t *d_G, uint32_t col0, uint32_t n_cols, uint8_t *d_out, hipStream_t st);
int launch_pad_tail(LayoutDev lay, uint64_t v_end, uint64_t vcol_begin, uint64_t vcol_end, int8_t *d_G,
                    hipStream_t st);
int launch_pad_tail_cursor(LayoutDev lay, const uint64_t *d_cursor, int8_t *d_G, hipStream_t st);

size_t lz4_slot_bytes(int neblock);
int launch_lz4_blocks(const uint8_t *d_src, const uint8_t *d_planes, PlanesGeom pg, uint64_t n_chunks, uint64_t chunk_nbytes, int typesize,
                      int blocksize, uint8_t *d_scratch, size_t slot_bytes, uint32_t *d_csize, int clevel, uint32_t *d_flags, uint32_t tag,
                      hipStream_t st);
int launch_lz4_bitplanes(const uint8_t *d_src, bool planes, PlanesGeom pg, uint64_t n_blocks, uint8_t *d_scratch, size_t slot_bytes, uint32_t *d_csize,
                         int depth, uint32_t *d_flags, uint32_t tag, hipStream_t st);
int launch_frame(const uint8_t *d_scratch, size_t slot_bytes, const uint32_t *d_csize, const uint8_t *d_src, const uint8_t *d_planes,
                 PlanesGeom pg, uint64_t n_chunks, uint64_t chunk_nbytes, int typesize, int blocksize, int format,
                 uint32_t *d_bstart, uint64_t *d_chunk_csize, uint8_t *d_dst, uint64_t dst_cap,
                 uint64_t *d_chunk_off, uint32_t *d_chunk_flags, hipStream_t st);
int launch_decode(const uint8_t *d_src, const uint64_t *d_chunk_off, uint64_t n_chunks, uint64_t chunk_nbytes,
                  int typesize, int blocksize, uint8_t *d_dst, unsigned long long *d_bad, hipStream_t st);
int launch_decode_sel(const hhgt_block_sel *d_sel, uint32_t n_sel, uint64_t chunk_nbytes, int typesize, int blocksize,
                      uint8_t *d_dst, unsigned long long *d_bad, hipStream_t st);
int launch_count_alleles(const hhgt_count_sel *d_sel, uint32_t n_sel, uint32_t sc, uint32_t vc, int blocksize,
                         uint32_t *d_counts, uint64_t n_out, unsigned long long *d_bad, hipStream_t st);
int launch_count_samples(const hhgt_sample_sel *d_sel, uint32_t n_sel, uint32_t sc, uint32_t vc, int blocksize,
                         const uint32_t *d_vmask, uint64_t vmask_words, uint32_t *d_counts, uint64_t n_out,
                         unsigned long long *d_bad, hipStream_t st);
int launch_genotype_planes(const hhgt_plane_sel *d_sel, uint32_t n_sel, uint32_t sc, uint32_t vc, int blocksize,
                           const uint32_t *d_vmask, uint64_t vmask_words, uint32_t *d_planes, uint64_t n_rows,
                           uint64_t row_words, unsigned long long *d_bad, hipStream_t st);
int launch_pair_counts(const uint32_t *d_planes, uint32_t n_rows, uint64_t row_words, uint64_t w_lo, uint64_t w_hi,
                       uint32_t *d_table, hipStream_t st);
int launch_grm(const uint32_t *d_planes, uint32_t n_rows, uint64_t row_words, uint64_t w_lo, uint64_t w_hi, const float *d_z,
               double *d_table, hipStream_t st);
int launch_variant_planes(const uint32_t *d_planes, uint32_t n_rows, uint64_t row_words, uint64_t w_lo, uint64_t w_hi,
                          uint32_t *d_vplanes, hipStream_t st);
int launch_ld_counts(const uint32_t *d_vplanes, uint64_t n_var, uint64_t sw, uint32_t window, uint32_t *d_table,
                     hipStream_t st);
uint32_t ld_walk_words(uint32_t window);
int launch_ld_exceeds(const uint32_t *d_table, uint64_t n_var, uint32_t window, double r2, uint64_t *d_bits, hipStream_t st);
int launch_ld_walk(const uint64_t *d_bits, uint64_t n_var, uint32_t window, uint8_t *d_keep, hipStream_t st);
int launch_assoc_sums(const uint32_t *d_vplanes, uint64_t n_var, uint64_t sw, const double *d_w, uint32_t n_cols,
                      double *d_sums, hipStream_t st);
int launch_inflate(const uint8_t *d_src, uint64_t src_bytes, const uint64_t *d_comp_off, const uint32_t *d_comp_len,
                   const uint64_t *d_out_off, const uint32_t *d_isize, uint64_t n_members, uint8_t *d_dst,
                   uint64_t dst_bytes, uint32_t *d_status, const uint32_t *d_crc32, const uint32_t *d_x2n, hipStream_t st);
void crc32_x2n_table(uint32_t *t );

static inline __host__ __device__ uint64_t layout_offset(const LayoutDev &L, uint32_t s, uint64_t v)
{
    uint64_t vcol = v / L.Vc, vin = v - vcol * L.Vc;
    if (L.ring) vcol %= L.ring;
    uint32_t scol = (L.sc_log2 >= 31) ? 0u : (s >> L.sc_log2);
    uint32_t sin = s - scol * L.Sc;
    return (((vcol * L.n_sc + scol) * L.Sc + sin) * L.Vc + vin) * 2ull;
}
```

### haplohyped_varawareml_amd/csrc/index.hip

```cpp
#include "common.h"

typedef uint32_t u32x4_unaligned __attribute__((ext_vector_type(4), aligned(1)));
typedef uint32_t u32x4_t __attribute__((ext_vector_type(4)));

__device__ __forceinline__ uint32_t nl_mask4(uint32_t x)
{
    uint32_t t = x ^ 0x0A0A0A0Au;
    uint32_t z = ~(((t & 0x7F7F7F7Fu) + 0x7F7F7F7Fu) | t | 0x7F7F7F7Fu);
    return (((z >> 7) * 0x01020408u) >> 24) & 0xFu;
}

__global__ __launch_bounds__(256) void k_index_newlines(const uint8_t *__restrict__ text, uint64_t n,
                                                        uint32_t *__restrict__ slots,
                                                        uint32_t *__restrict__ counts, uint32_t n_regions,
                                                        DevCounters *cnt)
{
    HHGT_WAVE_PRIO();
    const uint32_t lane = threadIdx.x & 63u;
    const uint32_t r = blockIdx.x * 4u + (threadIdx.x >> 6);
    if (r >= n_regions) return;
    const bool virt = n > 0 && text[n - 1] != '\n';
    const uint64_t rbase = (uint64_t)r * INDEX_REGION;
    uint32_t *my = slots + (size_t)r * INDEX_CAP;
    uint32_t wcount = 0;
    bool overflow = false;
    uint32_t masks[INDEX_REGION / 1024];
#pragma unroll
    for (int it = 0; it < (int)(INDEX_REGION / 1024); ++it) {
        uint64_t g0 = rbase + (uint64_t)it * 1024u + lane * 16u;
        uint32_t m = 0;
        if (g0 + 16 <= n) {
            const u32x4_t v4 = __builtin_nontemporal_load(reinterpret_cast<const u32x4_t *>(text + g0));
            uint4 v = make_uint4(v4.x, v4.y, v4.z, v4.w);
            m = nl_mask4(v.x) | (nl_mask4(v.y) << 4) | (nl_mask4(v.z) << 8) | (nl_mask4(v.w) << 12);
        } else if (g0 <= n) {
            for (int j = 0; j < 16; ++j) {
                uint64_t g = g0 + j;
                if (g < n) {
                    if (text[g] == '\n') m |= 1u << j;
                } else if (g == n && virt)
                    m |= 1u << j;
            }
        }
        masks[it] = m;
    }
#pragma unroll
    for (int it = 0; it < (int)(INDEX_REGION / 1024); ++it) {
        uint32_t m = masks[it];
        if (__ballot(m != 0) == 0ull) continue;
        uint32_t c = __popc(m);
        uint32_t inc = c;
#pragma unroll
        for (int d = 1; d < 64; d <<= 1) {
            uint32_t t = __shfl_up(inc, d, 64);
            if (lane >= (uint32_t)d) inc += t;
        }
        uint32_t idx = wcount + inc - c;
        uint32_t g0 = (uint32_t)(rbase + (uint64_t)it * 1024u + lane * 16u);
        while (m) {
            int j = __ffs(m) - 1;
            m &= m - 1;
            if (idx < INDEX_CAP) my[idx] = g0 + (uint32_t)j;
            else overflow = true;
            ++idx;
        }
        wcount += __shfl(inc, 63, 64);
    }
    if (__ballot(overflow) != 0ull && lane == 0) atomicAdd(&cnt->err_density, 1ull);
    if (lane == 0) counts[r] = wcount < INDEX_CAP ? wcount : INDEX_CAP;
}

__device__ __forceinline__ uint32_t eq_mask4(uint32_t x, uint32_t c4)
{
    const uint32_t t = x ^ c4;
    const uint32_t z = ~(((t & 0x7F7F7F7Fu) + 0x7F7F7F7Fu) | t | 0x7F7F7F7Fu);
    return (((z >> 7) * 0x01020408u) >> 24) & 0xFu;
}

__device__ __forceinline__ uint32_t eq_mask16(const u32x4_t &v, uint32_t c4)
{
    return eq_mask4(v.x, c4) | (eq_mask4(v.y, c4) << 4) | (eq_mask4(v.z, c4) << 8) | (eq_mask4(v.w, c4) << 12);
}

__device__ __forceinline__ uint32_t head_byte(const u32x4_t &v, uint32_t off)
{
    const uint32_t q = (off >> 2) & 3u;
    const uint32_t d = q == 0u ? v.x : (q == 1u ? v.y : (q == 2u ? v.z : v.w));
    return ((uint32_t)__builtin_amdgcn_readlane((int)d, (int)(off >> 4)) >> (8u * (off & 3u))) & 0xFFu;
}

__device__ __forceinline__ uint32_t head_kth(uint32_t m16, uint32_t cum, uint32_t k)
{
    const unsigned long long b = __builtin_amdgcn_ballot_w64(cum < k && cum + (uint32_t)__popc(m16) >= k);
    const int l = __builtin_ctzll(b);
    uint32_t m = (uint32_t)__builtin_amdgcn_readlane((int)m16, l);
    const uint32_t r = k - (uint32_t)__builtin_amdgcn_readlane((int)cum, l);
    for (uint32_t i = 1; i < r; ++i) m &= m - 1u;
    return 16u * (uint32_t)l + (uint32_t)__builtin_ctz(m);
}

#ifndef WALK_BATCH
#define WALK_BATCH 1
#endif
#ifndef WALK_PF
#define WALK_PF 0
#endif
template <int U, bool WALK>
__global__ __launch_bounds__(256) void k_index_hop(const uint8_t *__restrict__ text, uint64_t n, uint32_t *__restrict__ slots,
                                                   uint32_t *__restrict__ counts, uint32_t n_regions, uint32_t skip, uint32_t S,
                                                   DevCounters *cnt, uint32_t HOP_K)
{
    HHGT_WAVE_PRIO();
    const uint32_t lane = threadIdx.x & 63u;
    const uint32_t w = (uint32_t)__builtin_amdgcn_readfirstlane((int)(blockIdx.x * 4u + (threadIdx.x >> 6)));
    const uint32_t r_first = w * HOP_K;
    if (r_first >= n_regions) return;
    const uint32_t r_cnt = n_regions - r_first < HOP_K ? n_regions - r_first : HOP_K;
    const bool virt = n > 0 && text[n - 1] != '\n';
    const uint64_t beg = (uint64_t)r_first * INDEX_REGION;
    uint64_t endw = beg + (uint64_t)r_cnt * INDEX_REGION;
    if (endw > n + 1) endw = n + 1;
    const uint64_t last_term = virt ? n : n - 1;
    uint32_t cntv = 0;
    bool overflow = false;
    uint64_t pos = beg;
    uint64_t cand = 0, fb = 0;
    bool have_cand = false;
    uint64_t est_len = 0, pf_wb = 0;
    bool pf_valid = false;
    u32x4_t pf = u32x4_t{0u, 0u, 0u, 0u};
    auto record = [&](uint64_t q) {
        const uint32_t rr = (uint32_t)(q / INDEX_REGION), local = rr - r_first;
        const uint32_t c = (uint32_t)__builtin_amdgcn_readlane((int)cntv, (int)local);
        if (c < INDEX_CAP) {
            if (lane == 0) slots[(size_t)rr * INDEX_CAP + c] = (uint32_t)q;
        } else
            overflow = true;
        cntv += lane == local ? 1u : 0u;
    };
    bool no_batch = false, bat_off = false;
    uint32_t bat_fail = 0;
    uint64_t head_p = 0;
    bool cand_batch = false;
    bool rehead = false;
    while (have_cand || pos < endw) {
        if (WALK && WALK_BATCH && have_cand && !no_batch && !bat_off && est_len != 0ull && cand >= 40ull && cand + 3ull * est_len + 216ull <= n) {
            const uint32_t g = lane >> 4, li = lane & 15u;
            const uint64_t L0 = est_len;
            const uint8_t *wbase = text + (cand - 40ull);
            const uint64_t voff = (uint64_t)g * L0 + 16ull * li;
            const u32x4_t v = *reinterpret_cast<const u32x4_unaligned *>(wbase + voff);
            const uint32_t nlm = eq_mask16(v, 0x0A0A0A0Au), tbm = eq_mask16(v, 0x09090909u);
            const unsigned long long nlb = __builtin_amdgcn_ballot_w64(nlm != 0u);
            uint32_t og[4];
            bool vg[4];
#pragma unroll
            for (int k = 0; k < 4; ++k) {
                const uint32_t mg = (uint32_t)(nlb >> (16 * k)) & 0xFFFFu;
                vg[k] = mg != 0u;
                const int fl = 16 * k + __builtin_ctz(mg | 0x10000u);
                og[k] = 16u * ((uint32_t)fl & 15u) + (uint32_t)__builtin_ctz((uint32_t)__builtin_amdgcn_readlane((int)nlm, fl & 63) | 0x10000u);
            }
            const uint32_t o = g == 0u ? og[0] : (g == 1u ? og[1] : (g == 2u ? og[2] : og[3]));
            const uint32_t l0 = 16u * li;
            const uint32_t keep = l0 > o ? 0xFFFFu : (l0 + 15u <= o ? 0u : (0xFFFFu << (o - l0 + 1u)) & 0xFFFFu);
            const unsigned long long nl2 = __builtin_amdgcn_ballot_w64((nlm & keep) != 0u);
            const uint32_t tk = tbm & keep, tc = (uint32_t)__popc(tk);
            uint32_t incl = tc;
            incl += (uint32_t)__builtin_amdgcn_update_dpp(0, (int)incl, 0x111, 0xf, 0xf, false);
            incl += (uint32_t)__builtin_amdgcn_update_dpp(0, (int)incl, 0x112, 0xf, 0xf, false);
            incl += (uint32_t)__builtin_amdgcn_update_dpp(0, (int)incl, 0x114, 0xf, 0xf, false);
            incl += (uint32_t)__builtin_amdgcn_update_dpp(0, (int)incl, 0x118, 0xf, 0xf, false);
            const uint32_t cum = incl - tc;
            const bool has9 = cum < 9u && incl >= 9u;
            uint32_t m9 = tk;
            const uint32_t r1 = 8u - cum;
#pragma unroll
            for (uint32_t i = 0; i < 8u; ++i) m9 = i < r1 ? (m9 & (m9 - 1u)) : m9;
            const uint32_t j9 = (uint32_t)__builtin_ctz(m9 | 0x10000u) & 15u;
            const uint32_t pw = (uint32_t)__builtin_amdgcn_update_dpp(0, (int)v.w, 0x111, 0xf, 0xf, false);
            const uint32_t ptb = (uint32_t)__builtin_amdgcn_update_dpp(0, (int)tbm, 0x111, 0xf, 0xf, false);
            const uint32_t tb20 = (tbm << 4) | (ptb >> 12);
            const bool tab8 = ((tb20 >> (j9 + 1u)) & 1u) != 0u;
            const uint32_t ix = j9 + 2u, di = ix >> 2;
            const uint32_t w0 = di == 0u ? pw : (di == 1u ? v.x : (di == 2u ? v.y : (di == 3u ? v.z : v.w)));
            const uint32_t w1 = di == 0u ? v.x : (di == 1u ? v.y : (di == 2u ? v.z : v.w));
            const uint32_t gt2 = __builtin_amdgcn_alignbyte(w1, w0, ix & 3u) & 0xFFFFu;
            const bool ok9 = has9 && tab8 && gt2 == 0x5447u;
            const uint32_t t9 = l0 + j9;
            const unsigned long long b9 = __builtin_amdgcn_ballot_w64(ok9);
            uint64_t expected = cand, fbx = fb, exp_head = head_p;
            bool exp_batch = cand_batch;
            bool stop = false, handed = false;
            uint32_t advanced = 0;
#pragma unroll
            for (int k = 0; k < 4; ++k) {
                if (stop || handed) continue;
                const uint64_t nlpos = cand - 40ull + (uint64_t)k * L0 + og[k];
                const bool cr = vg[k] && og[k] != 0u && head_byte(v, 256u * (uint32_t)k + og[k] - 1u) == '\r';
                if (!vg[k] || nlpos != expected || cr) {
                    handed = true;
                    continue;
                }
                exp_head = expected;
                exp_batch = true;
                if (expected >= endw) {
                    stop = true;
                    continue;
                }
                const uint32_t bits = (uint32_t)(b9 >> (16 * k)) & 0xFFFFu;
                if (bits == 0u || ((nl2 >> (16 * k)) & 0xFFFFull) != 0ull) {
                    have_cand = false;
                    pos = expected;
                    handed = true;
                    expected = ~0ull;
                    continue;
                }
                record(expected);
                ++advanced;
                const int l9 = 16 * k + __builtin_ctz(bits);
                const uint32_t t9s = (uint32_t)__builtin_amdgcn_readlane((int)t9, l9);
                const uint64_t soff = cand - 40ull + (uint64_t)k * L0 + t9s + 1ull;
                const uint64_t nxt = soff + 4ull * S - 1ull;
                est_len = nxt - expected;
                expected = nxt;
                fbx = soff + 2ull * S - 17ull;
            }
            if (stop) break;
            if (expected != ~0ull) {
                if (expected > last_term) {
                    have_cand = false;
                    pos = fbx;
                    if (pos > last_term) pos = last_term;
                } else {
                    cand = expected;
                    fb = fbx > last_term ? last_term : fbx;
                    have_cand = true;
                }
                head_p = exp_head;
                cand_batch = exp_batch;
            }
            no_batch = handed;
            bat_fail = advanced ? 0u : bat_fail + 1u;
            bat_off = bat_fail >= 2u;
            continue;
        }
        no_batch = false;
        bool found = false, nb_have = false, have_head = false;
        uint32_t nb_reg = 0, ho = 15u;
        uint64_t p = 0;
        u32x4_t hd = u32x4_t{0u, 0u, 0u, 0u};
        if (WALK && have_cand) {
            have_cand = false;
            uint32_t c15 = 0, c14 = 0;
            const bool use_pf = pf_valid && cand >= pf_wb + 15ull && cand <= pf_wb + 79ull;
            pf_valid = false;
            if (use_pf || cand + 1009ull <= n) {
                if (use_pf) {
                    hd = pf;
                    ho = (uint32_t)(cand - pf_wb);
                } else
                    hd = *reinterpret_cast<const u32x4_unaligned *>(text + (cand - 15ull) + 16ull * lane);
                const uint64_t pred = cand + est_len;
                if (WALK_PF && est_len != 0ull && pred + 977ull <= n && cand < endw) {
                    pf_wb = pred - 47ull;
                    pf = *reinterpret_cast<const u32x4_unaligned *>(text + pf_wb + 16ull * lane);
                    pf_valid = true;
                }
                c15 = head_byte(hd, ho);
                c14 = head_byte(hd, ho - 1u);
                have_head = true;
            } else if (cand < n) {
                c15 = text[cand];
                c14 = text[cand - 1];
            } else if (cand == n && virt) {
                c15 = 0x0Au;
                c14 = text[n - 1];
            }
            if (c15 == 0x0Au && c14 != '\r') {
                found = true;
                p = cand;
            } else if (cand_batch) {
                cand_batch = false;
                rehead = true;
                found = true;
                have_head = false;
                p = head_p;
            } else {
                pos = fb;
                continue;
            }
        } else {
        const uint64_t a0 = pos & ~15ull;
        uint32_t any[U];
        u32x4_t v[U];
#pragma unroll
        for (int u = 0; u < U; ++u) {
            const uint64_t g0 = a0 + (uint64_t)u * 1024u + lane * 16u;
            uint32_t f = 0;
            v[u] = u32x4_t{0u, 0u, 0u, 0u};
            if (g0 + 16 <= n) {
                v[u] = __builtin_nontemporal_load(reinterpret_cast<const u32x4_t *>(text + g0));
                const uint32_t d[4] = {v[u].x, v[u].y, v[u].z, v[u].w};
#pragma unroll
                for (int q = 0; q < 4; ++q) {
                    const uint32_t t = d[q] ^ 0x0A0A0A0Au;
                    f |= (t - 0x01010101u) & ~t & 0x80808080u;
                }
            } else if (g0 <= n) {
                uint32_t d[4] = {0x20202020u, 0x20202020u, 0x20202020u, 0x20202020u};
                for (int j = 0; j < 16; ++j) {
                    const uint64_t g = g0 + j;
                    uint32_t ch = 0x20u;
                    if (g < n) ch = text[g];
                    else if (g == n && virt) ch = 0x0Au;
                    d[j >> 2] = (d[j >> 2] & ~(0xFFu << (8 * (j & 3)))) | (ch << (8 * (j & 3)));
                    if (ch == 0x0Au) f = 1u;
                }
                v[u] = u32x4_t{d[0], d[1], d[2], d[3]};
            }
            if (g0 + 16 <= pos) f = 0;
            any[u] = f;
        }
#pragma unroll
        for (int u = 0; u < U; ++u) {
            if (found) continue;
            unsigned long long b = __builtin_amdgcn_ballot_w64(any[u] != 0u);
            while (b != 0ull && !found) {
                const int l = __builtin_ctzll(b);
                b &= b - 1ull;
                const uint32_t x0 = (uint32_t)__builtin_amdgcn_readlane((int)v[u].x, l), x1 = (uint32_t)__builtin_amdgcn_readlane((int)v[u].y, l);
                const uint32_t x2 = (uint32_t)__builtin_amdgcn_readlane((int)v[u].z, l), x3 = (uint32_t)__builtin_amdgcn_readlane((int)v[u].w, l);
                uint32_t m = nl_mask4(x0) | (nl_mask4(x1) << 4) | (nl_mask4(x2) << 8) | (nl_mask4(x3) << 12);
                const uint64_t g0 = a0 + (uint64_t)u * 1024u + (uint64_t)l * 16u;
                if (g0 < pos) m &= ~((1u << (uint32_t)(pos - g0)) - 1u);
                if (m) {
                    found = true;
                    const uint32_t j = (uint32_t)__builtin_ctz(m);
                    p = g0 + j;
                    if (j < 15u && g0 + 16 <= n) {
                        const uint32_t k = j + 1u, dw = k >> 2;
                        const uint32_t xd = dw == 0u ? x0 : (dw == 1u ? x1 : (dw == 2u ? x2 : x3));
                        nb_reg = (xd >> (8u * (k & 3u))) & 0xFFu;
                        nb_have = true;
                    }
                }
            }
        }
        if (!found) {
            pos = a0 + (uint64_t)U * 1024u;
            continue;
        }
        }
        if (!rehead) {
            if (p >= endw) break;
            record(p);
        } else
            no_batch = true;
        rehead = false;
        bool hopped = false;
        if (WALK) {
            if (!have_head && p >= 15ull && p + 1009ull <= n) {
                hd = *reinterpret_cast<const u32x4_unaligned *>(text + (p - 15ull) + 16ull * lane);
                have_head = true;
            }
            if (have_head) {
                const uint64_t wb = p - (uint64_t)ho;
                const uint32_t nb = head_byte(hd, ho + 1u);
                const uint32_t l0 = 16u * lane;
                const uint32_t keep = l0 > ho ? 0xFFFFu : (l0 + 15u <= ho ? 0u : (0xFFFFu << (ho - l0 + 1u)) & 0xFFFFu);
                if (nb == '#' || nb == 0x0Au) {
                    pos = p + 1;
                    hopped = true;
                } else {
                    const uint32_t nlm = eq_mask16(hd, 0x0A0A0A0Au) & keep;
                    const unsigned long long nlb = __builtin_amdgcn_ballot_w64(nlm != 0u);
                    if (nlb != 0ull) {
                        const int l = __builtin_ctzll(nlb);
                        pos = wb + 16ull * (uint64_t)l + (uint64_t)__builtin_ctz((uint32_t)__builtin_amdgcn_readlane((int)nlm, l));
                        hopped = true;
                    } else {
                        const uint32_t tbm = eq_mask16(hd, 0x09090909u) & keep;
                        const uint32_t tc = (uint32_t)__popc(tbm);
                        const uint32_t incl = wave_scan_sum_dpp(tc, lane);
                        const uint32_t total = (uint32_t)__builtin_amdgcn_readlane((int)incl, 63);
                        if (total >= 9u) {
                            const uint32_t t8 = head_kth(tbm, incl - tc, 8u), t9 = head_kth(tbm, incl - tc, 9u);
                            const uint64_t soff = wb + t9 + 1ull;
                            const uint64_t lo = soff + 2ull * S - 17ull;
                            const bool gt = t9 - t8 == 3u && head_byte(hd, t8 + 1u) == 'G' && head_byte(hd, t8 + 2u) == 'T';
                            if (gt && soff + 4ull * S - 1ull <= last_term) {
                                cand = soff + 4ull * S - 1ull;
                                fb = lo;
                                have_cand = true;
                                est_len = cand - p;
                                head_p = p;
                                cand_batch = false;
                            } else {
                                pos = lo;
                            }
                            hopped = true;
                        }
                    }
                }
            }
        }
        if (!hopped) {
            uint32_t nb = 0x0Au;
            if (nb_have) nb = nb_reg;
            else if (p + 1 < n) nb = text[p + 1];
            pos = p + 1 + ((nb == '#' || nb == 0x0Au || nb == '\r') ? 0u : skip);
        }
        if (pos > last_term) pos = p + 1 > last_term ? p + 1 : last_term;
        if (have_cand && fb > last_term) fb = p + 1 > last_term ? p + 1 : last_term;
    }
    if (overflow && lane == 0) atomicAdd(&cnt->err_density, 1ull);
    if (lane < r_cnt) counts[r_first + lane] = cntv < INDEX_CAP ? cntv : INDEX_CAP;
}

__global__ __launch_bounds__(256) void k_compact_newlines(const uint32_t *__restrict__ slots,
                                                          const uint32_t *__restrict__ counts,
                                                          const uint32_t *__restrict__ prefix,
                                                          uint32_t n_regions, uint32_t *__restrict__ nl,
                                                          uint32_t max_lines)
{
    HHGT_WAVE_PRIO();
    uint32_t r = blockIdx.x * blockDim.x + threadIdx.x;
    if (r >= n_regions) return;
    uint32_t c = counts[r], p = prefix[r];
    const uint32_t *my = slots + (size_t)r * INDEX_CAP;
    for (uint32_t k = 0; k < c && p + k < max_lines; ++k) nl[p + k] = my[k];
}

__global__ __launch_bounds__(256) void k_parse_fixed(const uint8_t *__restrict__ text, uint64_t n,
                                                     const uint32_t *__restrict__ nl, const uint32_t *__restrict__ d_nlines,
                                                     uint32_t max_lines, const RegionFilter rfv, uint32_t S,
                                                     uint32_t *__restrict__ l_soff, uint32_t *__restrict__ l_lend,
                                                     uint32_t *__restrict__ l_pos, uint32_t *__restrict__ l_refalt,
                                                     uint32_t *__restrict__ l_flags, uint32_t *__restrict__ l_keep,
                                                     uint32_t *__restrict__ l_cnew, DevCounters *cnt, uint32_t hop_skip)
{
    HHGT_WAVE_PRIO();
    __shared__ uint32_t stage[256][17];
    const RegionFilter *rf = &rfv;
    const uint32_t i = blockIdx.x * blockDim.x + threadIdx.x;
    const uint32_t n_found = *d_nlines;
    const uint32_t n_lines = n_found < max_lines ? n_found : max_lines;
    if (i == 0) {
        cnt->n_lines = n_found;
        cnt->err_lines = n_found > max_lines ? (unsigned long long)(n_found - max_lines) : 0ull;
    }
    if (blockIdx.x * blockDim.x >= n_lines) {
        if (i < max_lines) l_keep[i] = l_cnew[i] = 0u;
        return;
    }
    uint32_t flags = 0;
    uint32_t s = 0, e = 0;
    bool staged = false;
    if (i < n_lines) {
        s = i ? nl[i - 1] + 1u : 0u;
        e = nl[i];
        staged = (uint64_t)s + 64ull <= n;
        if (staged) {
            u32x4_unaligned c[4];
#pragma unroll
            for (int k = 0; k < 4; ++k) c[k] = *reinterpret_cast<const u32x4_unaligned *>(text + s + 16 * k);
#pragma unroll
            for (int k = 0; k < 4; ++k) {
                stage[threadIdx.x][4 * k + 0] = c[k].x;
                stage[threadIdx.x][4 * k + 1] = c[k].y;
                stage[threadIdx.x][4 * k + 2] = c[k].z;
                stage[threadIdx.x][4 * k + 3] = c[k].w;
            }
        }
    }
    __syncthreads();
    const uint8_t *mine = reinterpret_cast<const uint8_t *>(stage[threadIdx.x]);
    auto rd = [&](uint32_t x) -> uint32_t { return (staged && x - s < 64u) ? (uint32_t)mine[x - s] : (uint32_t)text[x]; };
    uint32_t soff = 0, pos0 = 0, refalt = 0, gtidx = 0, stride = 0;
    if (i < n_lines) {
        if (e > s && rd(e - 1u) == '\r') --e;
        soff = e;
        if (e > s && rd(s) != '#') {
            flags = LF_RECORD;
            uint32_t fs[10];
            uint32_t nf = 0;
            uint32_t p = s;
            fs[0] = s;
            while (p < e && nf < 9) {
                if (rd(p) == '\t') fs[++nf] = p + 1;
                ++p;
            }
            bool bad = false;
            uint32_t fe[9];
#pragma unroll
            for (int k = 0; k < 9; ++k) fe[k] = (uint32_t)k < nf ? fs[k + 1] - 1u : e;
            if (nf < 7 || (S > 0 && nf < 9)) bad = true;
            if (!bad) {
                unsigned long long pos = 0;
                if (fe[1] == fs[1]) bad = true;
                for (uint32_t q = fs[1]; q < fe[1]; ++q) {
                    uint32_t c = rd(q);
                    if (c < '0' || c > '9') {
                        bad = true;
                        break;
                    }
                    pos = pos * 10ull + (c - '0');
                }
                bool in_region = true;
                if (!bad && rf->contig_len > 0) {
                    uint32_t cl = fe[0] - fs[0];
                    in_region = cl == (uint32_t)rf->contig_len;
                    for (uint32_t q = 0; in_region && q < cl; ++q)
                        in_region = rd(fs[0] + q) == (uint32_t)(uint8_t)rf->contig[q];
                    if (in_region && rf->has_range)
                        in_region = (long long)pos >= rf->beg && (long long)pos <= rf->end;
                }
                if (!bad) {
                    if (!in_region)
                        flags |= LF_DROP_REGION;
                    else {
                        uint32_t reflen = fe[3] - fs[3], altlen = fe[4] - fs[4];
                        uint32_t a = altlen >= 1 ? rd(fs[4]) : 0;
                        bool snp = reflen == 1 && altlen == 1 && (a == 'A' || a == 'C' || a == 'G' || a == 'T');
                        if (rf->keep_multi && reflen == 1 && altlen > 1 && (altlen & 1u)) {
                            snp = true;
                            for (uint32_t q = 0; snp && q < altlen; ++q) {
                                const uint32_t ch = rd(fs[4] + q);
                                snp = (q & 1u) ? ch == ',' : (ch == 'A' || ch == 'C' || ch == 'G' || ch == 'T');
                            }
                        }
                        if (!snp)
                            flags |= LF_DROP_FILTER;
                        else {
                            pos0 = (uint32_t)(pos - 1ull);
                            refalt = rd(fs[3]) | (a << 8);
                            if (S > 0) {
                                uint32_t q = fs[8], k = 0;
                                bool found = false;
                                while (q <= fe[8]) {
                                    uint32_t q2 = q;
                                    while (q2 < fe[8] && rd(q2) != ':') ++q2;
                                    if (q2 - q == 2 && rd(q) == 'G' && rd(q + 1u) == 'T') {
                                        found = true;
                                        break;
                                    }
                                    ++k;
                                    q = q2 + 1;
                                }
                                if (!found || k > 0xFFFu) bad = true;
                                gtidx = k;
                                soff = fs[9];
                                if (!bad) {
                                    flags |= LF_KEEP;
                                    if (k == 0 && fe[8] - fs[8] == 2 && e - soff == 4u * S - 1u) flags |= LF_FAST;
                                    else if (k == 0 && (e - soff + 1u) % S == 0u) {
                                        const uint32_t wd = (e - soff + 1u) / S;
                                        if (wd >= 5u && wd <= 8u) stride = wd;
                                    }
                                }
                            } else {
                                flags |= LF_KEEP;
                            }
                        }
                    }
                }
            }
            if (bad) flags = LF_RECORD | LF_MALFORMED;
            bool cnew = true;
            if (i > 0) {
                uint32_t ps = i > 1 ? nl[i - 2] + 1u : 0u;
                uint32_t pe = nl[i - 1];
                const bool pstaged = threadIdx.x > 0u && (uint64_t)ps + 64ull <= n;
                const uint8_t *prev = reinterpret_cast<const uint8_t *>(stage[threadIdx.x > 0u ? threadIdx.x - 1u : 0u]);
                auto rdp = [&](uint32_t x) -> uint32_t { return (pstaged && x - ps < 64u) ? (uint32_t)prev[x - ps] : (uint32_t)text[x]; };
                if (pe > ps && rdp(ps) != '#') {
                    uint32_t q = 0;
                    cnew = false;
                    for (;;) {
                        uint32_t a = fs[0] + q < e ? rd(fs[0] + q) : '\t';
                        uint32_t b = ps + q < pe ? rdp(ps + q) : '\t';
                        if (a != b) {
                            cnew = true;
                            break;
                        }
                        if (a == '\t') break;
                        ++q;
                    }
                }
            }
            if (cnew) flags |= LF_CHROM_NEW;
        }
    }
    if (hop_skip) {
        const uint32_t lane = threadIdx.x & 63u;
        const bool chk = (flags & LF_RECORD) && !(flags & (LF_KEEP | LF_MALFORMED));
        unsigned long long todo = __ballot(chk);
        while (todo != 0ull) {
            const int l = __builtin_ctzll(todo);
            todo &= todo - 1ull;
            const uint32_t ss = (uint32_t)__builtin_amdgcn_readlane((int)s, l), ee = (uint32_t)__builtin_amdgcn_readlane((int)e, l);
            const uint32_t hi = ee - ss < hop_skip ? ee : ss + hop_skip;
            uint32_t hit = 0;
            for (uint32_t x0 = ss + 16u * lane; x0 < hi; x0 += 8192u) {
                u32x4_t tv[8];
#pragma unroll
                for (int u = 0; u < 8; ++u) {
                    const uint32_t x = x0 + 1024u * (uint32_t)u;
                    tv[u] = u32x4_t{0u, 0u, 0u, 0u};
                    if (x < hi && (uint64_t)x + 16ull <= n) tv[u] = *reinterpret_cast<const u32x4_unaligned *>(text + x);
                }
#pragma unroll
                for (int u = 0; u < 8; ++u) {
                    const uint32_t x = x0 + 1024u * (uint32_t)u;
                    if (x >= hi) continue;
                    uint32_t d[4] = {tv[u].x, tv[u].y, tv[u].z, tv[u].w};
                    if ((uint64_t)x + 16ull > n)
                        for (uint32_t k = 0; k < 16u && (uint64_t)x + k < n; ++k) d[k >> 2] |= (uint32_t)text[x + k] << (8u * (k & 3u));
                    const uint32_t m = nl_mask4(d[0]) | (nl_mask4(d[1]) << 4) | (nl_mask4(d[2]) << 8) | (nl_mask4(d[3]) << 12);
                    hit |= hi - x >= 16u ? m : (m & ((1u << (hi - x)) - 1u));
                }
            }
            if (__ballot(hit != 0u) != 0ull && (int)lane == l) flags = (flags & LF_CHROM_NEW) | LF_RECORD | LF_MALFORMED;
        }
    }
    if (i < n_lines) {
        l_soff[i] = soff;
        l_lend[i] = e;
        l_pos[i] = pos0;
        l_refalt[i] = refalt | ((gtidx & 0xFFFu) << 16) | (stride << 28);
        l_flags[i] = flags;
        l_keep[i] = (flags & LF_KEEP) ? 1u : 0u;
        l_cnew[i] = (flags & LF_CHROM_NEW) ? 1u : 0u;
    } else if (i < max_lines) {
        l_keep[i] = l_cnew[i] = 0u;
    }
    __shared__ uint32_t s_stat[4];
    const uint32_t lane = threadIdx.x & 63u;
    if (threadIdx.x < 4u) s_stat[threadIdx.x] = 0u;
    __syncthreads();
    const uint32_t kinds[4] = {LF_RECORD, LF_DROP_REGION, LF_DROP_FILTER, LF_MALFORMED};
#pragma unroll
    for (int k = 0; k < 4; ++k) {
        const unsigned long long b = __ballot(flags & kinds[k]);
        if (lane == 0 && b) atomicAdd(&s_stat[k], (uint32_t)__popcll(b));
    }
    __syncthreads();
    if (threadIdx.x < 4u && s_stat[threadIdx.x]) {
        unsigned long long *dst = threadIdx.x == 0u ? &cnt->n_records : (threadIdx.x == 1u ? &cnt->n_drop_region : (threadIdx.x == 2u ? &cnt->n_drop_filter : &cnt->n_malformed));
        atomicAdd(dst, (unsigned long long)s_stat[threadIdx.x]);
    }
}

__global__ __launch_bounds__(256) void k_compact_kept(
    const uint8_t *__restrict__ text, uint64_t n, const uint32_t *__restrict__ nl, const uint32_t *__restrict__ d_nlines,
    uint32_t max_lines, const uint32_t *__restrict__ l_soff,
    const uint32_t *__restrict__ l_lend, const uint32_t *__restrict__ l_pos, const uint32_t *__restrict__ l_refalt,
    const uint32_t *__restrict__ l_flags, const uint32_t *__restrict__ l_kidx, const uint32_t *__restrict__ l_crun,
    uint32_t *__restrict__ k_soff, uint32_t *__restrict__ k_lend, uint32_t *__restrict__ k_meta,
    uint32_t *__restrict__ redo_list, uint32_t *__restrict__ redo_flag, uint64_t *__restrict__ run_first, uint8_t *__restrict__ run_names,
    uint32_t max_runs, const uint64_t *__restrict__ d_cursor, uint64_t v_capacity, uint32_t ring, uint32_t *__restrict__ d_start,
    uint32_t *__restrict__ d_stop, uint8_t *__restrict__ d_ref, uint8_t *__restrict__ d_alt, DevCounters *cnt, uint32_t strided)
{
    HHGT_WAVE_PRIO();
    const uint32_t i = blockIdx.x * blockDim.x + threadIdx.x;
    const uint32_t n_found = *d_nlines;
    const uint32_t n_lines = n_found < max_lines ? n_found : max_lines;
    if (i >= n_lines) return;
    const uint64_t v_base = *d_cursor;
    const uint32_t flags = l_flags[i];
    if (flags & LF_CHROM_NEW) {
        uint32_t rid = l_crun[i];
        if (rid < max_runs) {
            run_first[rid] = l_kidx[i];
            const uint32_t s0 = i ? nl[i - 1] + 1u : 0u;
            uint8_t *nm = run_names + (size_t)rid * 32u;
            uint32_t q = 0;
            for (; q < 31u && (uint64_t)s0 + q < n; ++q) {
                const uint8_t ch = text[s0 + q];
                if (ch == '\t' || ch == '\n') break;
                nm[q] = ch;
            }
            for (; q < 32u; ++q) nm[q] = 0;
        }
    }
    if (i == n_lines - 1) {
        cnt->n_kept = (unsigned long long)l_kidx[n_lines];
        cnt->n_chrom_runs = (unsigned long long)l_crun[n_lines];
    }
    const bool keep = (flags & LF_KEEP) != 0u;
    const bool slow = keep && !(flags & LF_FAST) && !(strided && (l_refalt[i < n_lines ? i : 0u] >> 28) != 0u);
    const unsigned long long sm = __ballot(slow);
    unsigned long long slot0 = 0ull;
    if (sm != 0ull) {
        const uint32_t lane = threadIdx.x & 63u;
        const int leader = __builtin_ctzll(sm);
        unsigned long long base = 0ull;
        if ((int)lane == leader) base = atomicAdd(&cnt->n_general, (unsigned long long)__popcll(sm));
        base = (unsigned long long)__shfl((long long)base, leader, 64);
        slot0 = base + (unsigned long long)__popcll(sm & ((1ull << lane) - 1ull));
    }
    if (!keep) return;
    const uint32_t k = l_kidx[i];
    uint64_t v = v_base + k;
    const uint32_t ra = l_refalt[i];
    k_soff[k] = l_soff[i];
    k_lend[k] = l_lend[i];
    k_meta[k] = (flags & LF_FAST) | ((ra >> 16) << 8);
    redo_flag[k] = 0u;
    if (slow) redo_list[slot0] = k;
    if (ring) v %= v_capacity;
    if (v < v_capacity) {
        uint32_t pos0 = l_pos[i];
        if (d_start) d_start[v] = pos0;
        if (d_stop) d_stop[v] = pos0 + 1u;
        if (d_ref) d_ref[v] = (uint8_t)(ra & 0xFFu);
        if (d_alt) d_alt[v] = (uint8_t)((ra >> 8) & 0xFFu);
    }
}

int index_mode_default()
{
    static const int m = [] {
        if (const char *e = getenv("HHGT_INDEX_MODE")) return atoi(e);
        if (const char *e = getenv("HHGT_INDEX_HOP")) return atoi(e) ? 2 : 0;
        return 2;
    }();
    return m < 0 ? 0 : (m > 2 ? 2 : m);
}

static uint32_t index_hop_skip(uint32_t min_line, int mode)
{
    if (mode < 0) mode = index_mode_default();
    return mode && min_line >= 1536u ? min_line - 16u : 0u;
}

int launch_index_newlines(const uint8_t *d_text, uint64_t n, uint32_t *d_slots, uint32_t *d_counts,
                          uint32_t n_regions, uint32_t min_line, uint32_t S, int mode, DevCounters *d_cnt, hipStream_t st)
{
    if (mode < 0) mode = index_mode_default();
    if (const uint32_t skip = index_hop_skip(min_line, mode)) {
        const bool walk = mode >= 2 && S > 0;
        const uint32_t k_walk = (n_regions + 8191u) / 8192u;
        uint32_t K = walk ? (k_walk < 6u ? 6u : k_walk) : 6u;
        K = K > 64u ? 64u : K;
#define HOP_LAUNCH(U, W)                                                                                                      \
    hipLaunchKernelGGL((k_index_hop<U, W>), dim3(((n_regions + K - 1) / K + 3) / 4), dim3(256), 0, st, d_text, n, d_slots, d_counts, \
                       n_regions, skip, S, d_cnt, K)
        if (min_line >= 4096u) {
            if (walk) HOP_LAUNCH(5, true);
            else HOP_LAUNCH(5, false);
        } else {
            if (walk) HOP_LAUNCH(3, true);
            else HOP_LAUNCH(3, false);
        }
#undef HOP_LAUNCH
        HIP_TRY(hipGetLastError());
        return HHGT_OK;
    }
    hipLaunchKernelGGL(k_index_newlines, dim3((n_regions + 3) / 4), dim3(256), 0, st, d_text, n, d_slots,
                       d_counts, n_regions, d_cnt);
    HIP_TRY(hipGetLastError());
    return HHGT_OK;
}

int launch_compact_newlines(const uint32_t *d_slots, const uint32_t *d_counts, const uint32_t *d_prefix,
                            uint32_t n_regions, uint32_t *d_nl, uint32_t max_lines, hipStream_t st)
{
    hipLaunchKernelGGL(k_compact_newlines, dim3((n_regions + 255) / 256), dim3(256), 0, st, d_slots, d_counts,
                       d_prefix, n_regions, d_nl, max_lines);
    HIP_TRY(hipGetLastError());
    return HHGT_OK;
}

int launch_parse_fixed(const uint8_t *d_text, uint64_t n, const uint32_t *d_nl, const uint32_t *d_nlines,
                       uint32_t max_lines, const RegionFilter &region, uint32_t S, const LineCols &l, int mode,
                       DevCounters *d_cnt, hipStream_t st)
{
    if (max_lines == 0) return HHGT_OK;
    if (mode < 0) mode = index_mode_default();
    uint32_t hop_skip = index_hop_skip(S ? 2u * S + 17u : 0u, mode);
    if (hop_skip && mode >= 2) hop_skip = 0xFFFFFFFFu;
    hipLaunchKernelGGL(k_parse_fixed, dim3((max_lines + 255) / 256), dim3(256), 0, st, d_text, n, d_nl, d_nlines,
                       max_lines, region, S, l.soff, l.lend, l.pos, l.refalt, l.flags, l.keep, l.cnew, d_cnt, hop_skip);
    HIP_TRY(hipGetLastError());
    return HHGT_OK;
}

int launch_compact_kept(const uint8_t *d_text, uint64_t n, const uint32_t *d_nl, const uint32_t *d_nlines, uint32_t max_lines,
                        const LineCols &l, const KeptCols &k, uint32_t max_runs, const uint64_t *d_cursor, uint64_t v_capacity,
                        uint32_t ring, uint32_t *d_start, uint32_t *d_stop, uint8_t *d_ref, uint8_t *d_alt, DevCounters *d_cnt,
                        bool strided, hipStream_t st)
{
    if (max_lines == 0) return HHGT_OK;
    hipLaunchKernelGGL(k_compact_kept, dim3((max_lines + 255) / 256), dim3(256), 0, st, d_text, n, d_nl, d_nlines, max_lines,
                       l.soff, l.lend, l.pos, l.refalt, l.flags, l.kidx, l.crun, k.soff, k.lend, k.meta, k.redo_list, k.redo_flag,
                       k.run_first, k.run_names, max_runs, d_cursor, v_capacity, ring, d_start, d_stop, d_ref, d_alt, d_cnt, strided ? 1u : 0u);
    HIP_TRY(hipGetLastError());
    return HHGT_OK;
}
```

### haplohyped_varawareml_amd/csrc/scan.hip

```cpp
#include "common.h"

#define SCAN_BLOCK 256
#define SCAN_ITEMS 8
#define SCAN_TILE (SCAN_BLOCK * SCAN_ITEMS)

__device__ __forceinline__ uint32_t wave_incl_scan(uint32_t v)
{
    const int lane = threadIdx.x & 63;
#pragma unroll
    for (int d = 1; d < 64; d <<= 1) {
        uint32_t t = __shfl_up(v, d, 64);
        if (lane >= d) v += t;
    }
    return v;
}

__device__ __forceinline__ uint32_t block_excl_scan(uint32_t v, uint32_t *total, uint32_t *sm )
{
    const int lane = threadIdx.x & 63, w = threadIdx.x >> 6;
    uint32_t inc = wave_incl_scan(v);
    if (lane == 63) sm[w] = inc;
    __syncthreads();
    uint32_t base = 0, tot = 0;
#pragma unroll
    for (int i = 0; i < SCAN_BLOCK / 64; ++i) {
        uint32_t x = sm[i];
        if (i < w) base += x;
        tot += x;
    }
    __syncthreads();
    *total = tot;
    return base + inc - v;
}

__global__ __launch_bounds__(SCAN_BLOCK) void k_scan_reduce(const uint32_t *__restrict__ in, uint64_t n,
                                                            uint32_t *__restrict__ partial)
{
    HHGT_WAVE_PRIO();
    __shared__ uint32_t sm[8];
    uint64_t base = (uint64_t)blockIdx.x * SCAN_TILE;
    uint32_t s = 0;
#pragma unroll
    for (int i = 0; i < SCAN_ITEMS; ++i) {
        uint64_t idx = base + (uint64_t)i * SCAN_BLOCK + threadIdx.x;
        if (idx < n) s += in[idx];
    }
    uint32_t tot;
    block_excl_scan(s, &tot, sm);
    if (threadIdx.x == 0) partial[blockIdx.x] = tot;
}

__global__ __launch_bounds__(SCAN_BLOCK) void k_scan_partials(uint32_t *partial, uint32_t nb)
{
    HHGT_WAVE_PRIO();
    __shared__ uint32_t sm[8];
    uint32_t carry = 0;
    for (uint32_t b0 = 0; b0 < nb; b0 += SCAN_BLOCK) {
        uint32_t i = b0 + threadIdx.x;
        uint32_t v = i < nb ? partial[i] : 0;
        uint32_t tot;
        uint32_t ex = block_excl_scan(v, &tot, sm);
        if (i < nb) partial[i] = carry + ex;
        carry += tot;
    }
    if (threadIdx.x == 0) partial[nb] = carry;
}

__global__ __launch_bounds__(SCAN_BLOCK) void k_scan_down(const uint32_t *__restrict__ in, uint64_t n,
                                                          const uint32_t *__restrict__ partial, uint32_t nb,
                                                          uint32_t *__restrict__ out)
{
    HHGT_WAVE_PRIO();
    __shared__ uint32_t sm[8];
    uint64_t base = (uint64_t)blockIdx.x * SCAN_TILE + (uint64_t)threadIdx.x * SCAN_ITEMS;
    uint32_t v[SCAN_ITEMS];
    uint32_t s = 0;
#pragma unroll
    for (int i = 0; i < SCAN_ITEMS; ++i) {
        uint64_t idx = base + i;
        v[i] = idx < n ? in[idx] : 0;
        s += v[i];
    }
    uint32_t tot;
    uint32_t ex = block_excl_scan(s, &tot, sm) + partial[blockIdx.x];
#pragma unroll
    for (int i = 0; i < SCAN_ITEMS; ++i) {
        uint64_t idx = base + i;
        if (idx < n) out[idx] = ex;
        ex += v[i];
    }
    if (blockIdx.x == 0 && threadIdx.x == 0) out[n] = partial[nb];
}

size_t scan_tmp_elems(uint64_t n) { return (size_t)((n + SCAN_TILE - 1) / SCAN_TILE) + 2; }

int launch_scan_exclusive_u32(const uint32_t *d_in, uint32_t *d_out, uint64_t n, uint32_t *d_tmp,
                              size_t tmp_elems, hipStream_t st)
{
    uint32_t nb = (uint32_t)((n + SCAN_TILE - 1) / SCAN_TILE);
    if (nb == 0) nb = 1;
    if (tmp_elems < (size_t)nb + 1) {
        hhgt_set_error("scan: tmp too small");
        return HHGT_ERR_ARG;
    }
    hipLaunchKernelGGL(k_scan_reduce, dim3(nb), dim3(SCAN_BLOCK), 0, st, d_in, n, d_tmp);
    hipLaunchKernelGGL(k_scan_partials, dim3(1), dim3(SCAN_BLOCK), 0, st, d_tmp, nb);
    hipLaunchKernelGGL(k_scan_down, dim3(nb), dim3(SCAN_BLOCK), 0, st, d_in, n, d_tmp, nb, d_out);
    HIP_TRY(hipGetLastError());
    return HHGT_OK;
}

template <int B>
__global__ __launch_bounds__(SCAN_BLOCK) void k_scan_reduce_n(const uint32_t *__restrict__ in0, const uint32_t *__restrict__ in1,
                                                              uint64_t n, uint32_t *__restrict__ partial, uint32_t nb)
{
    HHGT_WAVE_PRIO();
    __shared__ uint32_t sm[8];
    const uint32_t *ins[2] = {in0, in1};
    const uint64_t base = (uint64_t)blockIdx.x * SCAN_TILE;
#pragma unroll
    for (int b = 0; b < B; ++b) {
        uint32_t s = 0;
#pragma unroll
        for (int i = 0; i < SCAN_ITEMS; ++i) {
            const uint64_t idx = base + (uint64_t)i * SCAN_BLOCK + threadIdx.x;
            if (idx < n) s += ins[b][idx];
        }
        uint32_t tot;
        block_excl_scan(s, &tot, sm);
        if (threadIdx.x == 0) partial[(size_t)b * nb + blockIdx.x] = tot;
    }
}

template <int B>
__global__ __launch_bounds__(SCAN_BLOCK) void k_scan_down_n(const uint32_t *__restrict__ in0, const uint32_t *__restrict__ in1,
                                                            uint64_t n, const uint32_t *__restrict__ partial, uint32_t nb,
                                                            uint32_t *__restrict__ out0, uint32_t *__restrict__ out1)
{
    HHGT_WAVE_PRIO();
    __shared__ uint32_t sm[8];
    const uint32_t *ins[2] = {in0, in1};
    uint32_t *outs[2] = {out0, out1};
    const uint64_t base = (uint64_t)blockIdx.x * SCAN_TILE + (uint64_t)threadIdx.x * SCAN_ITEMS;
#pragma unroll
    for (int b = 0; b < B; ++b) {
        uint32_t pre = 0;
        for (uint32_t i = threadIdx.x; i < blockIdx.x; i += SCAN_BLOCK) pre += partial[(size_t)b * nb + i];
        uint32_t front;
        block_excl_scan(pre, &front, sm);
        uint32_t v[SCAN_ITEMS];
        uint32_t s = 0;
#pragma unroll
        for (int i = 0; i < SCAN_ITEMS; ++i) {
            const uint64_t idx = base + i;
            v[i] = idx < n ? ins[b][idx] : 0;
            s += v[i];
        }
        uint32_t tot;
        uint32_t ex = block_excl_scan(s, &tot, sm) + front;
#pragma unroll
        for (int i = 0; i < SCAN_ITEMS; ++i) {
            const uint64_t idx = base + i;
            if (idx < n) outs[b][idx] = ex;
            ex += v[i];
        }
        if (blockIdx.x == nb - 1 && threadIdx.x == 0) outs[b][n] = front + tot;
    }
}

#define SCAN_SHORT_MAX 2048u
int launch_scan_exclusive_u32_pair(const uint32_t *in_a, uint32_t *out_a, const uint32_t *in_b, uint32_t *out_b, uint64_t n,
                                   uint32_t *d_tmp, size_t tmp_elems, hipStream_t st)
{
    uint32_t nb = (uint32_t)((n + SCAN_TILE - 1) / SCAN_TILE);
    if (nb == 0) nb = 1;
    if (nb > SCAN_SHORT_MAX) {
        int rc = launch_scan_exclusive_u32(in_a, out_a, n, d_tmp, tmp_elems, st);
        if (rc == HHGT_OK && in_b) rc = launch_scan_exclusive_u32(in_b, out_b, n, d_tmp, tmp_elems, st);
        return rc;
    }
    if (tmp_elems < 2 * (size_t)nb) {
        hhgt_set_error("scan: tmp too small");
        return HHGT_ERR_ARG;
    }
    if (in_b) {
        hipLaunchKernelGGL(k_scan_reduce_n<2>, dim3(nb), dim3(SCAN_BLOCK), 0, st, in_a, in_b, n, d_tmp, nb);
        hipLaunchKernelGGL(k_scan_down_n<2>, dim3(nb), dim3(SCAN_BLOCK), 0, st, in_a, in_b, n, d_tmp, nb, out_a, out_b);
    } else {
        hipLaunchKernelGGL(k_scan_reduce_n<1>, dim3(nb), dim3(SCAN_BLOCK), 0, st, in_a, in_a, n, d_tmp, nb);
        hipLaunchKernelGGL(k_scan_down_n<1>, dim3(nb), dim3(SCAN_BLOCK), 0, st, in_a, in_a, n, d_tmp, nb, out_a, out_a);
    }
    HIP_TRY(hipGetLastError());
    return HHGT_OK;
}
```

Baseline: 152.1 million.

## Fuse prefix scans into index, compact and kept kernels via group totals

Result: faster. 153.9 million (median of 6 runs) (+1.2%).

```diff
diff --git a/haplohyped_varawareml_amd/csrc/api.hip b/haplohyped_varawareml_amd/csrc/api.hip
--- a/haplohyped_varawareml_amd/csrc/api.hip
+++ b/haplohyped_varawareml_amd/csrc/api.hip
@@ -63,24 +63,29 @@
         if (_rc != HHGT_OK) return _rc; \
     } while (0)
 
-int EncodeWs::ensure_index(uint32_t n_regions)
+int EncodeWs::ensure_index(uint32_t n_regions, hipStream_t st)
 {
     TRY(slots.ensure((size_t)n_regions * INDEX_CAP * 4));
     TRY(counts.ensure((size_t)n_regions * 4));
-    TRY(prefix.ensure(((size_t)n_regions + 1) * 4));
-    return ensure_scan(n_regions);
+    TRY(n_lines.ensure(4));
+    const size_t had = region_tot.cap;
+    TRY(region_tot.ensure((size_t)chain_groups(n_regions) * 4));
+    if (region_tot.cap != had) HIP_TRY(hipMemsetAsync(region_tot.p, 0, region_tot.cap, st));
+    return HHGT_OK;
 }
 
 int EncodeWs::ensure_lines(uint32_t max_lines)
 {
     const size_t nl4 = ((size_t)max_lines + 1) * 4;
     TRY(nl.ensure(nl4));
-    TRY(ensure_scan(max_lines));
     for (DevBuf &b : line) TRY(b.ensure(nl4));
+    TRY(line_tot.ensure(2 * (size_t)chain_groups(max_lines) * 4));
+    if (chain_scanned(max_lines)) {
+        for (DevBuf &b : scanned) TRY(b.ensure(nl4));
+        TRY(scan_tmp.ensure(2 * scan_tmp_elems(max_lines) * 4));
+    }
     return ensure_runs();
 }
-
-int EncodeWs::ensure_scan(uint64_t n) { return scan_tmp.ensure(2 * scan_tmp_elems(n) * 4); }
 
 int EncodeWs::ensure_runs()
 {
@@ -334,7 +339,8 @@
 }
 
 __global__ void k_encode_finish(DevCounters *cnt, uint64_t *cursor, const uint64_t *__restrict__ run_first,
-                                const uint8_t *__restrict__ run_names, uint64_t v_capacity, hhgt_encode_result *res)
+                                const uint8_t *__restrict__ run_names, uint64_t v_capacity, hhgt_encode_result *res,
+                                uint32_t *region_tot, uint32_t n_region_tot)
 {
     const uint32_t t = threadIdx.x;
     const uint64_t before = *cursor;
@@ -357,15 +363,17 @@
         res->n_lines_over = cnt->err_lines;
         res->err_density = cnt->err_density;
         res->v_capacity = v_capacity;
-        res->done = 1u;
         res->reserved = cnt->n_other > 0xFFFFFFFFull ? 0xFFFFFFFFu : (uint32_t)cnt->n_other;
     }
     const uint64_t n_runs = cnt->n_chrom_runs;
     if (t < HHGT_RESULT_RUNS) res->run_first[t] = t < n_runs ? run_first[t] : 0ull;
     for (uint32_t q = t; q < HHGT_RESULT_RUNS * 32u; q += blockDim.x)
         res->run_names[q >> 5][q & 31u] = (q >> 5) < n_runs ? (char)run_names[q] : 0;
+    __threadfence_system();
     __syncthreads();
+    if (t == 0) __hip_atomic_store(&res->done, 1u, __ATOMIC_RELEASE, __HIP_MEMORY_SCOPE_SYSTEM);
     if (t < sizeof(DevCounters) / 8u) reinterpret_cast<unsigned long long *>(cnt)[t] = 0ull;
+    for (uint32_t q = t; q < n_region_tot; q += blockDim.x) region_tot[q] = 0u;
 }
 
 __global__ void k_set_u64(uint64_t *p, uint64_t v) { *p = v; }
@@ -394,15 +402,23 @@
 
 static uint32_t index_regions(uint64_t nbytes) { return (uint32_t)((nbytes + 1 + INDEX_REGION - 1) / INDEX_REGION); }
 
+static int encode_begin_clean(hhgt_ctx *c, DevCounters *cnt, hipStream_t st)
+{
+    if (!c->counters_clean) {
+        HIP_TRY(hipMemsetAsync(cnt, 0, sizeof(DevCounters), st));
+        if (c->enc.region_tot.p) HIP_TRY(hipMemsetAsync(c->enc.region_tot.p, 0, c->enc.region_tot.cap, st));
+    }
+    c->counters_clean = false;
+    return HHGT_OK;
+}
+
 static int encode_stage_index(hhgt_ctx *c, const uint8_t *text, uint64_t nbytes, uint32_t n_regions, uint32_t min_line, uint32_t S,
                               DevCounters *cnt, hipStream_t st)
 {
     EncodeWs &w = c->enc;
-    TRY(w.ensure_index(n_regions));
-    TRY(launch_index_newlines(text, nbytes, w.slots.as<uint32_t>(), w.counts.as<uint32_t>(), n_regions, min_line, S, c->index_mode, cnt, st));
-    TRY(launch_scan_exclusive_u32_pair(w.counts.as<uint32_t>(), w.prefix.as<uint32_t>(), nullptr, nullptr, n_regions,
-                                       w.scan_tmp.as<uint32_t>(), w.scan_tmp.cap / 4, st));
-    return HHGT_OK;
+    TRY(w.ensure_index(n_regions, st));
+    return launch_index_newlines(text, nbytes, w.slots.as<uint32_t>(), w.counts.as<uint32_t>(), w.region_tot.as<uint32_t>(), n_regions,
+                                 min_line, S, c->index_mode, cnt, st);
 }
 
 static int encode_stage_rest(hhgt_ctx *c, const uint8_t *text, uint64_t nbytes, uint32_t n_regions, uint32_t max_lines,
@@ -411,18 +427,18 @@
 {
     EncodeWs &w = c->enc;
     TRY(w.ensure_lines(max_lines));
-    const uint32_t *nl = w.nl.as<uint32_t>(), *d_nlines = w.prefix.as<uint32_t>() + n_regions;
-    uint32_t *scan_tmp = w.scan_tmp.as<uint32_t>();
-    const LineCols l = w.line_cols();
+    const uint32_t *nl = w.nl.as<uint32_t>(), *d_nlines = w.n_lines.as<uint32_t>();
+    const LineCols l = w.line_cols(max_lines);
     const KeptCols k = w.kept_cols();
     TRY(timed(c, st, HHGT_STAGE_INDEX, [&] {
-        return launch_compact_newlines(w.slots.as<uint32_t>(), w.counts.as<uint32_t>(), w.prefix.as<uint32_t>(), n_regions,
-                                       w.nl.as<uint32_t>(), max_lines, st);
+        return launch_compact_newlines(w.slots.as<uint32_t>(), w.counts.as<uint32_t>(), w.region_tot.as<uint32_t>(), n_regions,
+                                       w.nl.as<uint32_t>(), max_lines, w.n_lines.as<uint32_t>(), st);
     }));
     if (max_lines == 0) return HHGT_OK;
     TRY(timed(c, st, HHGT_STAGE_FIXED, [&] {
         TRY(launch_parse_fixed(text, nbytes, nl, d_nlines, max_lines, rf, L.S, l, c->index_mode, cnt, st));
-        TRY(launch_scan_exclusive_u32_pair(l.keep, l.kidx, l.cnew, l.crun, max_lines, scan_tmp, w.scan_tmp.cap / 4, st));
+        if (chain_scanned(max_lines))
+            TRY(launch_scan_exclusive_u32_pair(l.keep, l.kidx, l.cnew, l.crun, max_lines, w.scan_tmp.as<uint32_t>(), w.scan_tmp.cap / 4, st));
         return launch_compact_kept(text, nbytes, nl, d_nlines, max_lines, l, k, MAX_CHROM_RUNS, d_cursor, L.v_capacity, L.ring,
                                    d_start, d_stop, d_ref, d_alt, cnt, d_P != nullptr, st);
     }));
@@ -439,13 +455,31 @@
     });
 }
 
-static int encode_finish(hhgt_ctx *c, uint64_t *d_cursor, const LayoutDev &L, DevCounters *cnt, hipStream_t st)
+static hhgt_encode_result *result_on_device(const hhgt_ctx *c, hhgt_encode_result *h_result)
+{
+    hipPointerAttribute_t a;
+    if (hipPointerGetAttributes(&a, h_result) != hipSuccess) {
+        (void)hipGetLastError();
+        return nullptr;
+    }
+    if (a.type != hipMemoryTypeHost || !a.devicePointer || a.device != c->device) return nullptr;
+    return static_cast<hhgt_encode_result *>(a.devicePointer);
+}
+
+static int encode_finish(hhgt_ctx *c, uint64_t *d_cursor, const LayoutDev &L, DevCounters *cnt, uint32_t n_regions,
+                         hhgt_encode_result *h_result, hipStream_t st)
 {
     TRY(c->enc.ensure_runs());
     const KeptCols k = c->enc.kept_cols();
+    hhgt_encode_result *staging = c->enc.result.as<hhgt_encode_result>();
+    hhgt_encode_result *direct = h_result ? result_on_device(c, h_result) : nullptr;
+    if (h_result) h_result->done = 0u;
     hipLaunchKernelGGL(k_encode_finish, dim3(1), dim3(256), 0, st, cnt, d_cursor, k.run_first, k.run_names,
-                       L.ring ? 0ull : L.v_capacity, c->enc.result.as<hhgt_encode_result>());
+                       L.ring ? 0ull : L.v_capacity, direct ? direct : staging, c->enc.region_tot.as<uint32_t>(),
+                       c->enc.region_tot.p ? chain_groups(n_regions) : 0u);
     HIP_TRY(hipGetLastError());
+    c->counters_clean = true;
+    if (h_result && !direct) HIP_TRY(hipMemcpyAsync(h_result, staging, sizeof(hhgt_encode_result), hipMemcpyDeviceToHost, st));
     return HHGT_OK;
 }
 
@@ -548,21 +582,14 @@
     if (planes) TRY(planes_check_layout(L));
     const uint8_t *text = static_cast<const uint8_t *>(d_text);
     DevCounters *cnt = c->counters.as<DevCounters>();
-    if (!c->counters_clean) HIP_TRY(hipMemsetAsync(cnt, 0, sizeof(DevCounters), st));
-    c->counters_clean = false;
+    TRY(encode_begin_clean(c, cnt, st));
     const uint32_t n_regions = index_regions(nbytes);
     if (nbytes) {
         TRY(timed(c, st, HHGT_STAGE_INDEX, [&] { return encode_stage_index(c, text, nbytes, n_regions, L.S ? 2u * L.S + 17u : 0u, L.S, cnt, st); }));
         TRY(encode_stage_rest(c, text, nbytes, n_regions, max_lines, rf, L, d_cursor, d_G, planes ? d_P : nullptr, d_start, d_stop, d_ref,
                               d_alt, cnt, st));
     }
-    TRY(encode_finish(c, d_cursor, L, cnt, st));
-    c->counters_clean = true;
-    if (h_result) {
-        h_result->done = 0u;
-        HIP_TRY(hipMemcpyAsync(h_result, c->enc.result.p, sizeof(hhgt_encode_result), hipMemcpyDeviceToHost, st));
-    }
-    return HHGT_OK;
+    return encode_finish(c, d_cursor, L, cnt, n_regions, h_result, st);
 }
 
 extern "C" int hhgt_encode_text_async(hhgt_ctx *c, const void *d_text, uint64_t nbytes, const char *region,
@@ -653,22 +680,20 @@
     const uint8_t *text = static_cast<const uint8_t *>(d_text);
     DevCounters *cnt = c->counters.as<DevCounters>();
     TRY(c->cursor.ensure(8));
-    HIP_TRY(hipMemsetAsync(cnt, 0, sizeof(DevCounters), st));
-    c->counters_clean = false;
+    TRY(encode_begin_clean(c, cnt, st));
     hipLaunchKernelGGL(k_set_u64, dim3(1), dim3(1), 0, st, c->cursor.as<uint64_t>(), v_base);
     const uint32_t n_regions = index_regions(nbytes);
     uint32_t n_lines = 0;
     {
         StageTimer t(c, st, HHGT_STAGE_INDEX);
         TRY(encode_stage_index(c, text, nbytes, n_regions, L.S ? 2u * L.S + 17u : 0u, L.S, cnt, st));
-        c->h_counters->n_lines = 0;
+        std::vector<uint32_t> totals(chain_groups(n_regions));
         c->h_counters->err_density = 0;
-        HIP_TRY(hipMemcpyAsync(&c->h_counters->n_lines, c->enc.prefix.as<uint32_t>() + n_regions, 4,
-                               hipMemcpyDeviceToHost, st));
+        HIP_TRY(hipMemcpyAsync(totals.data(), c->enc.region_tot.p, totals.size() * 4, hipMemcpyDeviceToHost, st));
         HIP_TRY(hipMemcpyAsync(&c->h_counters->err_density, &cnt->err_density, 8, hipMemcpyDeviceToHost, st));
         HIP_TRY(hipStreamSynchronize(st));
         t.stop();
-        n_lines = (uint32_t)(c->h_counters->n_lines & 0xFFFFFFFFull);
+        for (uint32_t x : totals) n_lines += x;
         if (c->h_counters->err_density) {
             hhgt_set_error("encode: more than %u newlines inside one %u-byte region (not VCF text)", INDEX_CAP,
                            INDEX_REGION);
@@ -679,11 +704,8 @@
     if (n_lines == 0) return HHGT_OK;
     TRY(encode_stage_rest(c, text, nbytes, n_regions, n_lines, rf, L, c->cursor.as<uint64_t>(), d_G, nullptr, d_start, d_stop, d_ref,
                           d_alt, cnt, st));
-    TRY(encode_finish(c, c->cursor.as<uint64_t>(), L, cnt, st));
-    c->counters_clean = true;
+    TRY(encode_finish(c, c->cursor.as<uint64_t>(), L, cnt, n_regions, c->h_result_pinned, st));
     hhgt_encode_result *hr = &c->h_result;
-    hr->done = 0u;
-    HIP_TRY(hipMemcpyAsync(c->h_result_pinned, c->enc.result.p, sizeof(hhgt_encode_result), hipMemcpyDeviceToHost, st));
     HIP_TRY(hipStreamSynchronize(st));
     *hr = *c->h_result_pinned;
     if (stats) *stats = hr->stats;
@@ -887,9 +909,9 @@
     HIP_TRY(hipSetDevice(c->device));
     if (text_bytes) {
         const uint32_t n_regions = index_regions(text_bytes);
-        TRY(c->enc.ensure_scan(n_regions > max_lines ? n_regions : max_lines));
-        TRY(c->enc.ensure_index(n_regions));
+        TRY(c->enc.ensure_index(n_regions, nullptr));
         TRY(c->enc.ensure_lines(max_lines));
+        HIP_TRY(hipStreamSynchronize(nullptr));
     }
     if (n_chunks) {
         TRY(check_codec_args(chunk_nbytes, typesize, blocksize, HHGT_BLOSC2));
diff --git a/haplohyped_varawareml_amd/csrc/common.h b/haplohyped_varawareml_amd/csrc/common.h
--- a/haplohyped_varawareml_amd/csrc/common.h
+++ b/haplohyped_varawareml_amd/csrc/common.h
@@ -25,6 +25,35 @@
     const uint32_t t2 = (uint32_t)__builtin_amdgcn_readlane((int)x, 47) + t1;
     const uint32_t row = lane >> 4;
     return x + (row == 0u ? 0u : (row == 1u ? t0 : (row == 2u ? t1 : t2)));
+}
+
+__device__ __forceinline__ uint32_t wave_incl_scan(uint32_t v)
+{
+    const int lane = threadIdx.x & 63;
+#pragma unroll
+    for (int d = 1; d < 64; d <<= 1) {
+        uint32_t t = __shfl_up(v, d, 64);
+        if (lane >= d) v += t;
+    }
+    return v;
+}
+
+__device__ __forceinline__ uint32_t block_excl_scan(uint32_t v, uint32_t *total, uint32_t *sm )
+{
+    const int lane = threadIdx.x & 63, w = threadIdx.x >> 6;
+    uint32_t inc = wave_incl_scan(v);
+    if (lane == 63) sm[w] = inc;
+    __syncthreads();
+    uint32_t base = 0, tot = 0;
+#pragma unroll
+    for (int i = 0; i < 4; ++i) {
+        uint32_t x = sm[i];
+        if (i < w) base += x;
+        tot += x;
+    }
+    __syncthreads();
+    *total = tot;
+    return base + inc - v;
 }
 #endif
 
@@ -131,8 +160,15 @@
     template <typename T> T *as() const { return reinterpret_cast<T *>(p); }
 };
 
+#define CHAIN_GROUP 256u
+#define CHAIN_FANIN_MAX 2048u
+static_assert(((0xFFFFFFF0ull + 1 + INDEX_REGION - 1) / INDEX_REGION + CHAIN_GROUP - 1) / CHAIN_GROUP <= CHAIN_FANIN_MAX,
+              "the region totals of the largest text block must stay inside the fan-in bound");
+static inline uint32_t chain_groups(uint32_t n) { return (n + CHAIN_GROUP - 1u) / CHAIN_GROUP; }
+static inline bool chain_scanned(uint32_t max_lines) { return chain_groups(max_lines) > CHAIN_FANIN_MAX; }
+
 struct LineCols {
-    uint32_t *soff, *lend, *pos, *refalt, *flags, *keep, *kidx, *cnew, *crun;
+    uint32_t *soff, *lend, *pos, *refalt, *flags, *tot, *keep, *kidx, *cnew, *crun;
 };
 struct KeptCols {
     uint32_t *soff, *lend, *meta, *redo_list, *redo_flag;
@@ -141,26 +177,34 @@
 };
 
 struct EncodeWs {
-    DevBuf slots, counts, prefix, nl, scan_tmp;
-    enum { L_SOFF, L_LEND, L_POS, L_REFALT, L_FLAGS, L_KEEP, L_KIDX, L_CNEW, L_CRUN, K_SOFF, K_LEND, K_META, REDO_LIST, REDO_FLAG, N_LINE };
+    DevBuf slots, counts, nl, scan_tmp;
+    DevBuf region_tot;
+    DevBuf n_lines;
+    DevBuf line_tot;
+    enum { L_SOFF, L_LEND, L_POS, L_REFALT, L_FLAGS, K_SOFF, K_LEND, K_META, REDO_LIST, REDO_FLAG, N_LINE };
+    enum { S_KEEP, S_KIDX, S_CNEW, S_CRUN, N_SCANNED };
     DevBuf line[N_LINE];
+    DevBuf scanned[N_SCANNED];
     DevBuf run_first, run_names;
     DevBuf result;
-    int ensure_index(uint32_t n_regions);
+    int ensure_index(uint32_t n_regions, hipStream_t st);
     int ensure_lines(uint32_t max_lines);
-    int ensure_scan(uint64_t n);
     int ensure_runs();
     template <typename F> void each(F f)
     {
-        for (DevBuf *b : {&slots, &counts, &prefix, &nl, &scan_tmp, &run_first, &run_names, &result}) f(*b);
+        for (DevBuf *b : {&slots, &counts, &nl, &scan_tmp, &region_tot, &n_lines, &line_tot, &run_first, &run_names, &result}) f(*b);
         for (DevBuf &b : line) f(b);
+        for (DevBuf &b : scanned) f(b);
     }
     uint32_t *col(int i) const { return line[i].as<uint32_t>(); }
-    LineCols line_cols() const
+    LineCols line_cols(uint32_t max_lines) const
     {
         LineCols l;
         l.soff = col(L_SOFF), l.lend = col(L_LEND), l.pos = col(L_POS), l.refalt = col(L_REFALT), l.flags = col(L_FLAGS);
-        l.keep = col(L_KEEP), l.kidx = col(L_KIDX), l.cnew = col(L_CNEW), l.crun = col(L_CRUN);
+        l.tot = line_tot.as<uint32_t>();
+        const bool sc = chain_scanned(max_lines);
+        l.keep = sc ? scanned[S_KEEP].as<uint32_t>() : nullptr, l.kidx = sc ? scanned[S_KIDX].as<uint32_t>() : nullptr;
+        l.cnew = sc ? scanned[S_CNEW].as<uint32_t>() : nullptr, l.crun = sc ? scanned[S_CRUN].as<uint32_t>() : nullptr;
         return l;
     }
     KeptCols kept_cols() const
@@ -223,11 +267,11 @@
                                    uint32_t *d_tmp, size_t tmp_elems, hipStream_t st);
 size_t scan_tmp_elems(uint64_t n);
 
-int launch_index_newlines(const uint8_t *d_text, uint64_t n, uint32_t *d_slots, uint32_t *d_counts,
+int launch_index_newlines(const uint8_t *d_text, uint64_t n, uint32_t *d_slots, uint32_t *d_counts, uint32_t *d_region_tot,
                           uint32_t n_regions, uint32_t min_line, uint32_t S, int mode, DevCounters *d_cnt, hipStream_t st);
 int index_mode_default();
-int launch_compact_newlines(const uint32_t *d_slots, const uint32_t *d_counts, const uint32_t *d_prefix,
-                            uint32_t n_regions, uint32_t *d_nl, uint32_t max_lines, hipStream_t st);
+int launch_compact_newlines(const uint32_t *d_slots, const uint32_t *d_counts, const uint32_t *d_region_tot,
+                            uint32_t n_regions, uint32_t *d_nl, uint32_t max_lines, uint32_t *d_nlines, hipStream_t st);
 int launch_parse_fixed(const uint8_t *d_text, uint64_t n, const uint32_t *d_nl, const uint32_t *d_nlines,
                        uint32_t max_lines, const RegionFilter &region, uint32_t S, const LineCols &l, int mode,
                        DevCounters *d_cnt, hipStream_t st);
diff --git a/haplohyped_varawareml_amd/csrc/index.hip b/haplohyped_varawareml_amd/csrc/index.hip
--- a/haplohyped_varawareml_amd/csrc/index.hip
+++ b/haplohyped_varawareml_amd/csrc/index.hip
@@ -12,8 +12,8 @@
 
 __global__ __launch_bounds__(256) void k_index_newlines(const uint8_t *__restrict__ text, uint64_t n,
                                                         uint32_t *__restrict__ slots,
-                                                        uint32_t *__restrict__ counts, uint32_t n_regions,
-                                                        DevCounters *cnt)
+                                                        uint32_t *__restrict__ counts, uint32_t *__restrict__ region_tot,
+                                                        uint32_t n_regions, DevCounters *cnt)
 {
     HHGT_WAVE_PRIO();
     const uint32_t lane = threadIdx.x & 63u;
@@ -67,7 +67,11 @@
         wcount += __shfl(inc, 63, 64);
     }
     if (__ballot(overflow) != 0ull && lane == 0) atomicAdd(&cnt->err_density, 1ull);
-    if (lane == 0) counts[r] = wcount < INDEX_CAP ? wcount : INDEX_CAP;
+    if (lane == 0) {
+        const uint32_t c = wcount < INDEX_CAP ? wcount : INDEX_CAP;
+        counts[r] = c;
+        if (c) atomicAdd(&region_tot[r / CHAIN_GROUP], c);
+    }
 }
 
 __device__ __forceinline__ uint32_t eq_mask4(uint32_t x, uint32_t c4)
@@ -107,8 +111,8 @@
 #endif
 template <int U, bool WALK>
 __global__ __launch_bounds__(256) void k_index_hop(const uint8_t *__restrict__ text, uint64_t n, uint32_t *__restrict__ slots,
-                                                   uint32_t *__restrict__ counts, uint32_t n_regions, uint32_t skip, uint32_t S,
-                                                   DevCounters *cnt, uint32_t HOP_K)
+                                                   uint32_t *__restrict__ counts, uint32_t *__restrict__ region_tot, uint32_t n_regions,
+                                                   uint32_t skip, uint32_t S, DevCounters *cnt, uint32_t HOP_K)
 {
     HHGT_WAVE_PRIO();
     const uint32_t lane = threadIdx.x & 63u;
@@ -415,19 +419,35 @@
         if (have_cand && fb > last_term) fb = p + 1 > last_term ? p + 1 : last_term;
     }
     if (overflow && lane == 0) atomicAdd(&cnt->err_density, 1ull);
-    if (lane < r_cnt) counts[r_first + lane] = cntv < INDEX_CAP ? cntv : INDEX_CAP;
-}
-
-__global__ __launch_bounds__(256) void k_compact_newlines(const uint32_t *__restrict__ slots,
-                                                          const uint32_t *__restrict__ counts,
-                                                          const uint32_t *__restrict__ prefix,
-                                                          uint32_t n_regions, uint32_t *__restrict__ nl,
-                                                          uint32_t max_lines)
+    const uint32_t mine = lane < r_cnt ? (cntv < INDEX_CAP ? cntv : INDEX_CAP) : 0u;
+    if (lane < r_cnt) counts[r_first + lane] = mine;
+    const uint32_t g0 = r_first / CHAIN_GROUP;
+    const uint32_t split = (g0 + 1u) * CHAIN_GROUP - r_first;
+    const uint32_t a = lane < split ? mine : 0u;
+    const uint32_t sum_a = (uint32_t)__builtin_amdgcn_readlane((int)wave_scan_sum_dpp(a, lane), 63);
+    const uint32_t sum_b = (uint32_t)__builtin_amdgcn_readlane((int)wave_scan_sum_dpp(mine - a, lane), 63);
+    if (lane == 0) {
+        if (sum_a) atomicAdd(&region_tot[g0], sum_a);
+        if (sum_b) atomicAdd(&region_tot[g0 + 1u], sum_b);
+    }
+}
+
+__global__ __launch_bounds__(CHAIN_GROUP) void k_compact_newlines(const uint32_t *__restrict__ slots,
+                                                                  const uint32_t *__restrict__ counts,
+                                                                  const uint32_t *__restrict__ region_tot,
+                                                                  uint32_t n_regions, uint32_t *__restrict__ nl,
+                                                                  uint32_t max_lines, uint32_t *__restrict__ d_nlines)
 {
     HHGT_WAVE_PRIO();
-    uint32_t r = blockIdx.x * blockDim.x + threadIdx.x;
-    if (r >= n_regions) return;
-    uint32_t c = counts[r], p = prefix[r];
+    __shared__ uint32_t sm[8];
+    const uint32_t r = blockIdx.x * CHAIN_GROUP + threadIdx.x;
+    uint32_t pre = 0;
+    for (uint32_t g = threadIdx.x; g < blockIdx.x; g += CHAIN_GROUP) pre += region_tot[g];
+    uint32_t front, own;
+    block_excl_scan(pre, &front, sm);
+    const uint32_t c = r < n_regions ? counts[r] : 0u;
+    const uint32_t p = front + block_excl_scan(c, &own, sm);
+    if (blockIdx.x == gridDim.x - 1u && threadIdx.x == 0u) *d_nlines = front + own;
     const uint32_t *my = slots + (size_t)r * INDEX_CAP;
     for (uint32_t k = 0; k < c && p + k < max_lines; ++k) nl[p + k] = my[k];
 }
@@ -437,9 +457,11 @@
                                                      uint32_t max_lines, const RegionFilter rfv, uint32_t S,
                                                      uint32_t *__restrict__ l_soff, uint32_t *__restrict__ l_lend,
                                                      uint32_t *__restrict__ l_pos, uint32_t *__restrict__ l_refalt,
-                                                     uint32_t *__restrict__ l_flags, uint32_t *__restrict__ l_keep,
-                                                     uint32_t *__restrict__ l_cnew, DevCounters *cnt, uint32_t hop_skip)
-{
+                                                     uint32_t *__restrict__ l_flags, uint32_t *__restrict__ l_tot,
+                                                     uint32_t *__restrict__ l_keep, uint32_t *__restrict__ l_cnew,
+                                                     DevCounters *cnt, uint32_t hop_skip)
+{
+    static_assert(CHAIN_GROUP == 256u, "one k_parse_fixed workgroup is one group of k_compact_kept's prefix");
     HHGT_WAVE_PRIO();
     __shared__ uint32_t stage[256][17];
     const RegionFilter *rf = &rfv;
@@ -451,7 +473,8 @@
         cnt->err_lines = n_found > max_lines ? (unsigned long long)(n_found - max_lines) : 0ull;
     }
     if (blockIdx.x * blockDim.x >= n_lines) {
-        if (i < max_lines) l_keep[i] = l_cnew[i] = 0u;
+        if (threadIdx.x == 0u) l_tot[blockIdx.x] = l_tot[gridDim.x + blockIdx.x] = 0u;
+        if (l_keep && i < max_lines) l_keep[i] = l_cnew[i] = 0u;
         return;
     }
     uint32_t flags = 0;
@@ -630,18 +653,18 @@
         l_pos[i] = pos0;
         l_refalt[i] = refalt | ((gtidx & 0xFFFu) << 16) | (stride << 28);
         l_flags[i] = flags;
+    }
+    if (l_keep && i < max_lines) {
         l_keep[i] = (flags & LF_KEEP) ? 1u : 0u;
         l_cnew[i] = (flags & LF_CHROM_NEW) ? 1u : 0u;
-    } else if (i < max_lines) {
-        l_keep[i] = l_cnew[i] = 0u;
-    }
-    __shared__ uint32_t s_stat[4];
+    }
+    __shared__ uint32_t s_stat[6];
     const uint32_t lane = threadIdx.x & 63u;
-    if (threadIdx.x < 4u) s_stat[threadIdx.x] = 0u;
+    if (threadIdx.x < 6u) s_stat[threadIdx.x] = 0u;
     __syncthreads();
-    const uint32_t kinds[4] = {LF_RECORD, LF_DROP_REGION, LF_DROP_FILTER, LF_MALFORMED};
-#pragma unroll
-    for (int k = 0; k < 4; ++k) {
+    const uint32_t kinds[6] = {LF_RECORD, LF_DROP_REGION, LF_DROP_FILTER, LF_MALFORMED, LF_KEEP, LF_CHROM_NEW};
+#pragma unroll
+    for (int k = 0; k < 6; ++k) {
         const unsigned long long b = __ballot(flags & kinds[k]);
         if (lane == 0 && b) atomicAdd(&s_stat[k], (uint32_t)__popcll(b));
     }
@@ -650,29 +673,56 @@
         unsigned long long *dst = threadIdx.x == 0u ? &cnt->n_records : (threadIdx.x == 1u ? &cnt->n_drop_region : (threadIdx.x == 2u ? &cnt->n_drop_filter : &cnt->n_malformed));
         atomicAdd(dst, (unsigned long long)s_stat[threadIdx.x]);
     }
-}
-
-__global__ __launch_bounds__(256) void k_compact_kept(
+    if (threadIdx.x == 4u) l_tot[blockIdx.x] = s_stat[4];
+    if (threadIdx.x == 5u) l_tot[gridDim.x + blockIdx.x] = s_stat[5];
+}
+
+template <bool SCANNED>
+__global__ __launch_bounds__(CHAIN_GROUP) void k_compact_kept(
     const uint8_t *__restrict__ text, uint64_t n, const uint32_t *__restrict__ nl, const uint32_t *__restrict__ d_nlines,
     uint32_t max_lines, const uint32_t *__restrict__ l_soff,
     const uint32_t *__restrict__ l_lend, const uint32_t *__restrict__ l_pos, const uint32_t *__restrict__ l_refalt,
-    const uint32_t *__restrict__ l_flags, const uint32_t *__restrict__ l_kidx, const uint32_t *__restrict__ l_crun,
+    const uint32_t *__restrict__ l_flags, const uint32_t *__restrict__ l_tot, const uint32_t *__restrict__ l_kidx,
+    const uint32_t *__restrict__ l_crun,
     uint32_t *__restrict__ k_soff, uint32_t *__restrict__ k_lend, uint32_t *__restrict__ k_meta,
     uint32_t *__restrict__ redo_list, uint32_t *__restrict__ redo_flag, uint64_t *__restrict__ run_first, uint8_t *__restrict__ run_names,
     uint32_t max_runs, const uint64_t *__restrict__ d_cursor, uint64_t v_capacity, uint32_t ring, uint32_t *__restrict__ d_start,
     uint32_t *__restrict__ d_stop, uint8_t *__restrict__ d_ref, uint8_t *__restrict__ d_alt, DevCounters *cnt, uint32_t strided)
 {
     HHGT_WAVE_PRIO();
-    const uint32_t i = blockIdx.x * blockDim.x + threadIdx.x;
+    const uint32_t i = blockIdx.x * CHAIN_GROUP + threadIdx.x;
     const uint32_t n_found = *d_nlines;
     const uint32_t n_lines = n_found < max_lines ? n_found : max_lines;
-    if (i >= n_lines) return;
+    if (blockIdx.x * CHAIN_GROUP >= n_lines) return;
+    const bool live = i < n_lines;
+    const uint32_t flags = live ? l_flags[i] : 0u;
+    uint32_t kidx, crun;
+    if (SCANNED) {
+        kidx = live ? l_kidx[i] : 0u;
+        crun = live ? l_crun[i] : 0u;
+    } else {
+        __shared__ uint32_t sm[8];
+        uint32_t pre_k = 0, pre_c = 0;
+        for (uint32_t g = threadIdx.x; g < blockIdx.x; g += CHAIN_GROUP) {
+            pre_k += l_tot[g];
+            pre_c += l_tot[gridDim.x + g];
+        }
+        uint32_t front_k, front_c, own;
+        block_excl_scan(pre_k, &front_k, sm);
+        block_excl_scan(pre_c, &front_c, sm);
+        const uint32_t ex = block_excl_scan(((flags & LF_KEEP) ? 1u : 0u) | ((flags & LF_CHROM_NEW) ? 0x10000u : 0u), &own, sm);
+        kidx = front_k + (ex & 0xFFFFu);
+        crun = front_c + (ex >> 16);
+    }
+    if (i == n_lines - 1) {
+        cnt->n_kept = (unsigned long long)kidx + ((flags & LF_KEEP) ? 1u : 0u);
+        cnt->n_chrom_runs = (unsigned long long)crun + ((flags & LF_CHROM_NEW) ? 1u : 0u);
+    }
     const uint64_t v_base = *d_cursor;
-    const uint32_t flags = l_flags[i];
     if (flags & LF_CHROM_NEW) {
-        uint32_t rid = l_crun[i];
+        uint32_t rid = crun;
         if (rid < max_runs) {
-            run_first[rid] = l_kidx[i];
+            run_first[rid] = kidx;
             const uint32_t s0 = i ? nl[i - 1] + 1u : 0u;
             uint8_t *nm = run_names + (size_t)rid * 32u;
             uint32_t q = 0;
@@ -684,12 +734,8 @@
             for (; q < 32u; ++q) nm[q] = 0;
         }
     }
-    if (i == n_lines - 1) {
-        cnt->n_kept = (unsigned long long)l_kidx[n_lines];
-        cnt->n_chrom_runs = (unsigned long long)l_crun[n_lines];
-    }
     const bool keep = (flags & LF_KEEP) != 0u;
-    const bool slow = keep && !(flags & LF_FAST) && !(strided && (l_refalt[i < n_lines ? i : 0u] >> 28) != 0u);
+    const bool slow = keep && !(flags & LF_FAST) && !(strided && (l_refalt[live ? i : 0u] >> 28) != 0u);
     const unsigned long long sm = __ballot(slow);
     unsigned long long slot0 = 0ull;
     if (sm != 0ull) {
@@ -701,7 +747,7 @@
         slot0 = base + (unsigned long long)__popcll(sm & ((1ull << lane) - 1ull));
     }
     if (!keep) return;
-    const uint32_t k = l_kidx[i];
+    const uint32_t k = kidx;
     uint64_t v = v_base + k;
     const uint32_t ra = l_refalt[i];
     k_soff[k] = l_soff[i];
@@ -735,7 +781,7 @@
     return mode && min_line >= 1536u ? min_line - 16u : 0u;
 }
 
-int launch_index_newlines(const uint8_t *d_text, uint64_t n, uint32_t *d_slots, uint32_t *d_counts,
+int launch_index_newlines(const uint8_t *d_text, uint64_t n, uint32_t *d_slots, uint32_t *d_counts, uint32_t *d_region_tot,
                           uint32_t n_regions, uint32_t min_line, uint32_t S, int mode, DevCounters *d_cnt, hipStream_t st)
 {
     if (mode < 0) mode = index_mode_default();
@@ -746,7 +792,7 @@
         K = K > 64u ? 64u : K;
 #define HOP_LAUNCH(U, W)                                                                                                      \
     hipLaunchKernelGGL((k_index_hop<U, W>), dim3(((n_regions + K - 1) / K + 3) / 4), dim3(256), 0, st, d_text, n, d_slots, d_counts, \
-                       n_regions, skip, S, d_cnt, K)
+                       d_region_tot, n_regions, skip, S, d_cnt, K)
         if (min_line >= 4096u) {
             if (walk) HOP_LAUNCH(5, true);
             else HOP_LAUNCH(5, false);
@@ -759,16 +805,16 @@
         return HHGT_OK;
     }
     hipLaunchKernelGGL(k_index_newlines, dim3((n_regions + 3) / 4), dim3(256), 0, st, d_text, n, d_slots,
-                       d_counts, n_regions, d_cnt);
+                       d_counts, d_region_tot, n_regions, d_cnt);
     HIP_TRY(hipGetLastError());
     return HHGT_OK;
 }
 
-int launch_compact_newlines(const uint32_t *d_slots, const uint32_t *d_counts, const uint32_t *d_prefix,
-                            uint32_t n_regions, uint32_t *d_nl, uint32_t max_lines, hipStream_t st)
-{
-    hipLaunchKernelGGL(k_compact_newlines, dim3((n_regions + 255) / 256), dim3(256), 0, st, d_slots, d_counts,
-                       d_prefix, n_regions, d_nl, max_lines);
+int launch_compact_newlines(const uint32_t *d_slots, const uint32_t *d_counts, const uint32_t *d_region_tot,
+                            uint32_t n_regions, uint32_t *d_nl, uint32_t max_lines, uint32_t *d_nlines, hipStream_t st)
+{
+    hipLaunchKernelGGL(k_compact_newlines, dim3(chain_groups(n_regions)), dim3(CHAIN_GROUP), 0, st, d_slots, d_counts,
+                       d_region_tot, n_regions, d_nl, max_lines, d_nlines);
     HIP_TRY(hipGetLastError());
     return HHGT_OK;
 }
@@ -781,8 +827,8 @@
     if (mode < 0) mode = index_mode_default();
     uint32_t hop_skip = index_hop_skip(S ? 2u * S + 17u : 0u, mode);
     if (hop_skip && mode >= 2) hop_skip = 0xFFFFFFFFu;
-    hipLaunchKernelGGL(k_parse_fixed, dim3((max_lines + 255) / 256), dim3(256), 0, st, d_text, n, d_nl, d_nlines,
-                       max_lines, region, S, l.soff, l.lend, l.pos, l.refalt, l.flags, l.keep, l.cnew, d_cnt, hop_skip);
+    hipLaunchKernelGGL(k_parse_fixed, dim3(chain_groups(max_lines)), dim3(CHAIN_GROUP), 0, st, d_text, n, d_nl, d_nlines,
+                       max_lines, region, S, l.soff, l.lend, l.pos, l.refalt, l.flags, l.tot, l.keep, l.cnew, d_cnt, hop_skip);
     HIP_TRY(hipGetLastError());
     return HHGT_OK;
 }
@@ -793,9 +839,14 @@
                         bool strided, hipStream_t st)
 {
     if (max_lines == 0) return HHGT_OK;
-    hipLaunchKernelGGL(k_compact_kept, dim3((max_lines + 255) / 256), dim3(256), 0, st, d_text, n, d_nl, d_nlines, max_lines,
-                       l.soff, l.lend, l.pos, l.refalt, l.flags, l.kidx, l.crun, k.soff, k.lend, k.meta, k.redo_list, k.redo_flag,
-                       k.run_first, k.run_names, max_runs, d_cursor, v_capacity, ring, d_start, d_stop, d_ref, d_alt, d_cnt, strided ? 1u : 0u);
+#define KEPT_LAUNCH(SCANNED)                                                                                                         \
+    hipLaunchKernelGGL(k_compact_kept<SCANNED>, dim3(chain_groups(max_lines)), dim3(CHAIN_GROUP), 0, st, d_text, n, d_nl, d_nlines, \
+                       max_lines, l.soff, l.lend, l.pos, l.refalt, l.flags, l.tot, l.kidx, l.crun, k.soff, k.lend, k.meta,          \
+                       k.redo_list, k.redo_flag, k.run_first, k.run_names, max_runs, d_cursor, v_capacity, ring, d_start, d_stop,   \
+                       d_ref, d_alt, d_cnt, strided ? 1u : 0u)
+    if (chain_scanned(max_lines)) KEPT_LAUNCH(true);
+    else KEPT_LAUNCH(false);
+#undef KEPT_LAUNCH
     HIP_TRY(hipGetLastError());
     return HHGT_OK;
 }
diff --git a/haplohyped_varawareml_amd/csrc/scan.hip b/haplohyped_varawareml_amd/csrc/scan.hip
--- a/haplohyped_varawareml_amd/csrc/scan.hip
+++ b/haplohyped_varawareml_amd/csrc/scan.hip
@@ -3,35 +3,6 @@
 #define SCAN_BLOCK 256
 #define SCAN_ITEMS 8
 #define SCAN_TILE (SCAN_BLOCK * SCAN_ITEMS)
-
-__device__ __forceinline__ uint32_t wave_incl_scan(uint32_t v)
-{
-    const int lane = threadIdx.x & 63;
-#pragma unroll
-    for (int d = 1; d < 64; d <<= 1) {
-        uint32_t t = __shfl_up(v, d, 64);
-        if (lane >= d) v += t;
-    }
-    return v;
-}
-
-__device__ __forceinline__ uint32_t block_excl_scan(uint32_t v, uint32_t *total, uint32_t *sm )
-{
-    const int lane = threadIdx.x & 63, w = threadIdx.x >> 6;
-    uint32_t inc = wave_incl_scan(v);
-    if (lane == 63) sm[w] = inc;
-    __syncthreads();
-    uint32_t base = 0, tot = 0;
-#pragma unroll
-    for (int i = 0; i < SCAN_BLOCK / 64; ++i) {
-        uint32_t x = sm[i];
-        if (i < w) base += x;
-        tot += x;
-    }
-    __syncthreads();
-    *total = tot;
-    return base + inc - v;
-}
 
 __global__ __launch_bounds__(SCAN_BLOCK) void k_scan_reduce(const uint32_t *__restrict__ in, uint64_t n,
                                                             uint32_t *__restrict__ partial)
@@ -176,20 +147,15 @@
     if (nb == 0) nb = 1;
     if (nb > SCAN_SHORT_MAX) {
         int rc = launch_scan_exclusive_u32(in_a, out_a, n, d_tmp, tmp_elems, st);
-        if (rc == HHGT_OK && in_b) rc = launch_scan_exclusive_u32(in_b, out_b, n, d_tmp, tmp_elems, st);
+        if (rc == HHGT_OK) rc = launch_scan_exclusive_u32(in_b, out_b, n, d_tmp, tmp_elems, st);
         return rc;
     }
     if (tmp_elems < 2 * (size_t)nb) {
         hhgt_set_error("scan: tmp too small");
         return HHGT_ERR_ARG;
     }
-    if (in_b) {
-        hipLaunchKernelGGL(k_scan_reduce_n<2>, dim3(nb), dim3(SCAN_BLOCK), 0, st, in_a, in_b, n, d_tmp, nb);
-        hipLaunchKernelGGL(k_scan_down_n<2>, dim3(nb), dim3(SCAN_BLOCK), 0, st, in_a, in_b, n, d_tmp, nb, out_a, out_b);
-    } else {
-        hipLaunchKernelGGL(k_scan_reduce_n<1>, dim3(nb), dim3(SCAN_BLOCK), 0, st, in_a, in_a, n, d_tmp, nb);
-        hipLaunchKernelGGL(k_scan_down_n<1>, dim3(nb), dim3(SCAN_BLOCK), 0, st, in_a, in_a, n, d_tmp, nb, out_a, out_a);
-    }
+    hipLaunchKernelGGL(k_scan_reduce_n<2>, dim3(nb), dim3(SCAN_BLOCK), 0, st, in_a, in_b, n, d_tmp, nb);
+    hipLaunchKernelGGL(k_scan_down_n<2>, dim3(nb), dim3(SCAN_BLOCK), 0, st, in_a, in_b, n, d_tmp, nb, out_a, out_b);
     HIP_TRY(hipGetLastError());
     return HHGT_OK;
 }
```
